# lbcb-sci/herro

Hardware: AMD Instinct MI355X
Metric: 4096-bp windows corrected/sec at batch=128 (higher is better)
Workload: dtype f16; 1 GPU; synthetic windows, 4096 bp, 32 overlaps each, batch=128, 1xMI355X per rank (BASELINE configs[2]); batch=128, window=4096, overlaps=32, batches_per_launch_group=32, streams_per_gpu=2, distinct_windows_cycled=16384, precision=5, total_windows=165760, strong_leg_windows=0

## Files before the change

### herro_amd/api.py

```python
from __future__ import annotations

import ctypes as C
import os
from dataclasses import dataclass

import numpy as np

_HERE = os.path.dirname(os.path.abspath(__file__))
LIB_PATH = os.environ.get("HERRO_LIB") or os.path.join(_HERE, "libherro_amd.so")
_LIB = None
DEFAULT_PRECISION = 4

EXPORTS = [
    "herro_version", "herro_create", "herro_destroy", "herro_last_error", "herro_set_stream", "herro_synchronize",
    "herro_encode_2bit", "herro_decode_2bit", "herro_set_reads", "herro_set_reads_packed", "herro_share_reads", "herro_load_model",
    "herro_set_precision", "herro_precision", "herro_clock_probe", "herro_calibration_error", "herro_debug_force_precision", "herro_model_describe", "herro_job_create", "herro_job_free", "herro_job_n_windows", "herro_job_skipped", "herro_job_featurize",
    "herro_job_infer", "herro_job_consensus", "herro_job_consensus_fetch", "herro_job_window_info", "herro_job_window_copy", "herro_job_window_logits",
    "herro_job_consensus_fasta", "herro_job_fasta", "herro_model_forward", "herro_timing_enable", "herro_timing_reset",
    "herro_timing_get", "herro_job_stats", "herro_debug_extract_windows",
    "herro_paf_parse", "herro_oec_read", "herro_paf_n_targets", "herro_paf_target_ids", "herro_paf_aln_off",
    "herro_paf_alignments", "herro_paf_free", "herro_name_index_create", "herro_name_index_free", "herro_paf_parse_indexed",
    "herro_oec_read_indexed", "herro_paf_parse_view", "herro_debug_host_ctx", "herro_debug_job_array", "herro_debug_tile_plan", "herro_debug_tile_plan_sib",
    "herro_debug_set_featurize_planes", "herro_debug_set_host_build", "herro_debug_job_dev_built", "herro_debug_job_rf", "herro_debug_job_cwd", "herro_debug_job_set_base_logits", "herro_debug_job_rf_fused", "herro_debug_job_rf_left", "herro_debug_e4m3", "herro_debug_sib_fault", "herro_debug_sib_retries", "herro_debug_base_row_votes", "herro_debug_vote5",
    "herro_pool_create", "herro_pool_destroy", "herro_pool_last_error", "herro_pool_size", "herro_pool_ctx", "herro_pool_set_reads", "herro_pool_load_model",
    "herro_pool_correct", "herro_pool_result", "herro_pool_groups_taken", "herro_pool_skipped", "herro_debug_pool_fake", "herro_job_create_status", "herro_host_register", "herro_host_unregister", "herro_debug_zero_copy_jobs",
    "herro_fastx_read", "herro_reads_count", "herro_reads_seq", "herro_reads_qual", "herro_reads_off", "herro_reads_ids",
    "herro_reads_descs", "herro_reads_free", "herro_write_window_features", "herro_job_write_features",
    "herro_paf_parse_coords", "herro_align_overlaps", "herro_aligned_alignments", "herro_aligned_scores", "herro_aligned_failed",
    "herro_aligned_free",
    "herro_align_overlaps_dev", "herro_aligned_dev_from_ops", "herro_aligned_dev_mirror", "herro_aligned_dev_n", "herro_aligned_dev_alignments", "herro_aligned_dev_scores",
    "herro_aligned_dev_n_ops", "herro_aligned_dev_failed", "herro_aligned_dev_cigar", "herro_aligned_dev_free", "herro_job_create_aligned",
    "herro_find_overlaps", "herro_overlaps_n", "herro_overlaps_n_targets", "herro_overlaps_target_ids", "herro_overlaps_aln_off",
    "herro_overlaps_alignments", "herro_overlaps_scores", "herro_overlaps_free", "herro_debug_sketch",
    "herro_extend_overlaps", "herro_extended_n", "herro_extended_alignments", "herro_extended_ext", "herro_extended_scores", "herro_extended_free",
    "herro_find_overlap_pairs", "herro_pairs_from_table", "herro_pairs_align", "herro_job_create_paired", "herro_pairs_n", "herro_pairs_primaries",
    "herro_pairs_chain_scores", "herro_pairs_ext", "herro_pairs_ext_scores", "herro_pairs_n_targets", "herro_pairs_target_ids", "herro_pairs_aln_off",
    "herro_pairs_rec_of_row", "herro_pairs_free",
    "herro_find_overlaps_core", "herro_find_overlap_pairs_core", "herro_pairs_from_table_core", "herro_pairs_n_rows",
]


class HerroError(RuntimeError):
    def __init__(self, code: int, msg: str):
        super().__init__(f"herro_amd error {code}: {msg}")
        self.code = code


class Alignment(C.Structure):
    _fields_ = [(n, C.c_uint32) for n in
                ("qid", "qlen", "qstart", "qend", "strand", "tid", "tlen", "tstart", "tend", "cigar_len")] + \
               [("cigar", C.c_void_p)]


ALN_DTYPE = np.dtype([("f", np.uint32, 10), ("p", np.uint64)], align=True)


def _aln_array(rows: np.ndarray, ncols: int = 9):
    n = len(rows)
    arr = (Alignment * max(n, 1))()
    view = np.frombuffer(arr, dtype=ALN_DTYPE, count=max(n, 1))
    if n:
        view["f"][:n, :ncols] = rows[:, :ncols]
    return arr, view


def _aln_rows(ptr, n: int, with_cigar_ptr: bool = False):
    rows, cig = np.zeros((n, 10), np.uint32), np.zeros(n, np.uint64)
    if n:
        view = np.frombuffer((Alignment * n).from_address(ptr), dtype=ALN_DTYPE, count=n)
        rows[:], cig[:] = view["f"], view["p"]
    return (rows, cig) if with_cigar_ptr else rows


def _job_or_raise(ctx: "Context", h, n_targets: int) -> "Job":
    if not h:
        msg = ctx._l.herro_last_error(ctx.h).decode(errors="replace")
        code = int(msg.rsplit("[code ", 1)[1].rstrip("]")) if "[code " in msg else -1
        raise HerroError(code, msg)
    return Job(ctx, h, n_targets)


PAIRS_NO_EXTEND = 1


class OverlapParams(C.Structure):
    _fields_ = [(n, C.c_uint32) for n in ("k", "w", "max_occ", "bandwidth", "max_gap", "min_score", "min_anchors", "reserved")]


class ExtendParams(C.Structure):
    _fields_ = [("zdrop", C.c_uint32), ("max_ext", C.c_uint32), ("reserved", C.c_uint32 * 2)]


class WindowInfo(C.Structure):
    _fields_ = [(n, C.c_uint32) for n in
                ("rid", "wid", "n_total_wins", "length", "n_alns", "n_overlaps", "n_supported", "win_len")]


def lib():
    global _LIB
    if _LIB is None:
        if not os.path.exists(LIB_PATH):
            raise RuntimeError(f"{LIB_PATH} not built — run __graft_entry__.build(); there is no CPU fallback")
        L = C.CDLL(LIB_PATH)
        vp, u32, u64, i32 = C.c_void_p, C.c_uint32, C.c_uint64, C.c_int
        L.herro_version.restype = C.c_char_p
# ... 106 lines not shown
        L.herro_aligned_free.argtypes = [vp]
        L.herro_align_overlaps_dev.argtypes = [vp, u32, vp, vp]
        L.herro_aligned_dev_from_ops.argtypes = [vp, u32, vp, vp, vp, vp]
        L.herro_aligned_dev_mirror.argtypes = [vp, vp, vp]
        for f in (L.herro_aligned_dev_n, L.herro_aligned_dev_failed):
            f.restype = u32
            f.argtypes = [vp]
        for f in (L.herro_aligned_dev_alignments, L.herro_aligned_dev_scores, L.herro_aligned_dev_n_ops):
            f.restype = vp
            f.argtypes = [vp]
        L.herro_aligned_dev_cigar.restype = C.c_int64
        L.herro_aligned_dev_cigar.argtypes = [vp, u32, vp, u64]
        L.herro_aligned_dev_free.restype = None
        L.herro_aligned_dev_free.argtypes = [vp]
        L.herro_job_create_aligned.restype = vp
        L.herro_job_create_aligned.argtypes = [vp, u32, vp, vp, vp, vp, u32]
        L.herro_find_overlaps.argtypes = [vp, vp, vp]
        for f in (L.herro_overlaps_n, L.herro_overlaps_n_targets):
            f.restype = u32
            f.argtypes = [vp]
        for f in (L.herro_overlaps_target_ids, L.herro_overlaps_aln_off, L.herro_overlaps_alignments, L.herro_overlaps_scores):
            f.restype = vp
            f.argtypes = [vp]
        L.herro_overlaps_free.restype = None
        L.herro_overlaps_free.argtypes = [vp]
        L.herro_extend_overlaps.argtypes = [vp, u32, vp, vp, vp]
        L.herro_extended_n.restype = u32
        L.herro_extended_n.argtypes = [vp]
        for f in (L.herro_extended_alignments, L.herro_extended_ext, L.herro_extended_scores):
            f.restype = vp
            f.argtypes = [vp]
        L.herro_extended_free.restype = None
        L.herro_extended_free.argtypes = [vp]
        L.herro_find_overlap_pairs.argtypes = [vp, vp, vp, u32, vp]
        L.herro_pairs_from_table.argtypes = [vp, u32, vp, vp, u32, vp, vp, vp, vp]
        L.herro_pairs_align.argtypes = [vp, vp, vp]
        L.herro_job_create_paired.restype = vp
        L.herro_job_create_paired.argtypes = [vp, vp, vp, u32]
        for f in (L.herro_pairs_n, L.herro_pairs_n_targets):
            f.restype = u32
            f.argtypes = [vp]
        for f in (L.herro_pairs_primaries, L.herro_pairs_chain_scores, L.herro_pairs_ext, L.herro_pairs_ext_scores, L.herro_pairs_target_ids,
                  L.herro_pairs_aln_off, L.herro_pairs_rec_of_row):
            f.restype = vp
            f.argtypes = [vp]
        L.herro_pairs_free.restype = None
        L.herro_pairs_free.argtypes = [vp]
        try:
            L.herro_find_overlaps_core.argtypes = [vp, vp, vp, vp]
            L.herro_find_overlap_pairs_core.argtypes = [vp, vp, vp, u32, vp, vp]
            L.herro_pairs_from_table_core.argtypes = [vp, u32, vp, vp, u32, vp, vp, u64, vp, vp]
            L.herro_pairs_n_rows.restype = u64
            L.herro_pairs_n_rows.argtypes = [vp]
        except AttributeError:
            if not os.environ.get("HERRO_LIB"):
                raise
        L.herro_debug_sketch.restype = C.c_int64
        L.herro_debug_sketch.argtypes = [vp, vp, vp, vp, vp, vp, u64]
        L.herro_debug_host_ctx.restype = vp
        L.herro_debug_host_ctx.argtypes = [u32, vp, vp]
        L.herro_debug_job_array.restype = C.c_int64
        L.herro_debug_job_array.argtypes = [vp, i32, vp, vp]
        L.herro_debug_set_featurize_planes.argtypes = [vp, i32]
        L.herro_debug_set_host_build.argtypes = [vp, i32]
        L.herro_debug_job_dev_built.argtypes = [vp]
        L.herro_debug_base_row_votes.argtypes = [vp, vp, vp, u32, vp, vp]
        L.herro_debug_vote5.restype = u32
        L.herro_debug_vote5.argtypes = [vp, u32]
        L.herro_debug_job_rf_fused.argtypes = [vp]
        L.herro_debug_job_rf_left.argtypes = [vp]
        L.herro_debug_sib_fault.argtypes = [vp]
        L.herro_debug_e4m3.argtypes = [C.c_float]
        L.herro_debug_e4m3.restype = C.c_uint32
        L.herro_debug_sib_retries.argtypes = [vp]
        L.herro_debug_job_rf.restype = C.c_int64
        L.herro_debug_job_rf.argtypes = [vp, u32, vp, u64]
        L.herro_debug_job_cwd.restype = C.c_int64
        L.herro_debug_job_cwd.argtypes = [vp, u32, vp, u64]
        L.herro_debug_job_set_base_logits.argtypes = [vp, vp, u64]
        L.herro_debug_tile_plan.restype = C.c_int64
        L.herro_debug_tile_plan.argtypes = [vp, u32, i32, u32, vp, vp, vp]
        L.herro_debug_tile_plan_sib.restype = i32
        L.herro_debug_tile_plan_sib.argtypes = [vp, u32, i32, u32, vp, vp, vp, vp]
        _LIB = L
    return _LIB


def encode_2bit(seq: bytes) -> np.ndarray:
    words = np.zeros((len(seq) + 31) // 32 + 1, np.uint64)
    buf = np.frombuffer(seq, np.uint8)
    n = lib().herro_encode_2bit(buf.ctypes.data if len(seq) else None, len(seq), words.ctypes.data)
    if n < 0:
        raise HerroError(int(n), "byte >= 128 in sequence")
    return words[:n].copy()


def decode_2bit(words: np.ndarray, length: int, start: int, end: int, rc: bool) -> bytes:
    words = np.ascontiguousarray(words, np.uint64)
    out = np.zeros(max(end - start, 0), np.uint8)
    r = lib().herro_decode_2bit(words.ctypes.data, length, start, end, int(rc), out.ctypes.data)
    if r:
        raise HerroError(r, "Out of bounds for 2-bit sequence decoding.")
    return out.tobytes()


def debug_extract_windows(row, cigar: bytes, n_windows: int, window_size: int) -> np.ndarray:
    a = Alignment()
    (a.qid, a.qlen, a.qstart, a.qend, a.strand, a.tid, a.tlen, a.tstart, a.tend) = (int(x) for x in row)
    buf = np.frombuffer(cigar + b"\0", np.uint8).copy()
    a.cigar_len, a.cigar = len(cigar), buf.ctypes.data
    out = np.zeros((65536, 8), np.uint64)
    err = C.create_string_buffer(512)
    n = lib().herro_debug_extract_windows(C.byref(a), n_windows, window_size, out.ctypes.data, len(out), err, 512)
    if n < 0:
        raise HerroError(int(n), err.value.decode())
    return out[:n].astype(np.int64)


def debug_tile_plan(counts, packed: bool = True, qmode: int = 0, n_cu: int = 256, bounds: bool = False):
    c = np.ascontiguousarray(counts, np.uint32)
    order = np.zeros(max(len(c), 1), np.uint32)
    n_half = C.c_uint32(0)
    tok = np.zeros(len(c) + 2, np.uint32)
    n = lib().herro_debug_tile_plan(c.ctypes.data, len(c), int(packed) | (qmode << 1), n_cu, order.ctypes.data, C.byref(n_half), tok.ctypes.data)
    if n < 0:
        raise HerroError(int(n), "herro_debug_tile_plan")
    out = (int(n), int(n_half.value), order[:len(c)]) if qmode else (int(n), order[:len(c)])
    return out + (tok[:int(n) + int(n_half.value) + 1],) if bounds else out


def debug_tile_plan_sib(counts, packed: bool = True, qmode: int = 1, n_cu: int = 256):
    c = np.ascontiguousarray(counts, np.uint32)
    order = np.zeros(max(len(c), 1), np.uint32)
    cap = int(((c.astype(np.int64) + 63) // 64).sum()) + 2
    n_tiles = np.zeros(3, np.uint32)
    tok = np.zeros(cap, np.uint32)
    grp = np.zeros(cap, np.uint32)
    rc = lib().herro_debug_tile_plan_sib(c.ctypes.data, len(c), int(packed) | (qmode << 1), n_cu, order.ctypes.data, n_tiles.ctypes.data, tok.ctypes.data, grp.ctypes.data)
    if rc < 0:
        raise HerroError(int(rc), "herro_debug_tile_plan_sib")
    nb, n64, n32 = (int(x) for x in n_tiles)
    return nb, n64, n32, order[:len(c)], tok[:nb + n64 + n32 + 1], grp[:nb]


class Pool:

    def __init__(self, device_ids, fake_us_per_aln=None):
        self._l = lib()
        if fake_us_per_aln is not None:
            us = np.ascontiguousarray(fake_us_per_aln, np.uint32)
            self.h = self._l.herro_debug_pool_fake(len(us), us.ctypes.data)
            self.n = len(us)
            if not self.h:
                raise HerroError(-1, "herro_debug_pool_fake")
            return
        ids = (C.c_int * len(device_ids))(*device_ids)
        self.h = self._l.herro_pool_create(ids, len(device_ids))
        if not self.h:
            raise HerroError(-1, self._l.herro_last_error(None).decode(errors="replace"))
        self.n = len(device_ids)

    def skipped(self) -> tuple[int, int]:
        a, t = C.c_uint64(0), C.c_uint64(0)
        self._chk(self._l.herro_pool_skipped(self.h, C.byref(a), C.byref(t)))
        return a.value, t.value

    def _chk(self, rc):
        if rc < 0:
            raise HerroError(int(rc), self._l.herro_pool_last_error(self.h).decode(errors="replace"))
        return rc

    def set_reads(self, seq, qual, off, name_class=None):
        seq, qual, off = np.ascontiguousarray(seq, np.uint8), np.ascontiguousarray(qual, np.uint8), np.ascontiguousarray(off, np.uint64)
        nc = None if name_class is None else np.ascontiguousarray(name_class, np.uint32)
        self._chk(self._l.herro_pool_set_reads(self.h, len(off) - 1, seq.ctypes.data, qual.ctypes.data, off.ctypes.data, None if nc is None else nc.ctypes.data))

    def load_model(self, path: str):
        self._chk(self._l.herro_pool_load_model(self.h, path.encode()))

    def set_precision(self, mode: int):
        for i in range(self.n):
            rc = self._l.herro_set_precision(self._l.herro_pool_ctx(self.h, i), mode)
            if rc:
                raise HerroError(rc, self._l.herro_last_error(self._l.herro_pool_ctx(self.h, i)).decode(errors="replace"))

    def correct(self, rids, rows, aln_off, cig_blob, cig_off, window_size: int, batch: int, read_ids, batch_mode: int = 1, group_targets: int = 1024):
        rids = np.ascontiguousarray(rids, np.uint32)
        aln_off = np.ascontiguousarray(aln_off, np.uint64)
        rows = np.ascontiguousarray(rows, np.uint32).reshape(-1, 10)
        blob = np.ascontiguousarray(cig_blob, np.uint8)
        m = len(rows)
        raw = np.zeros((max(m, 1), 12), np.uint32)
        if m:
            raw[:m, :10] = rows
            raw[:m, 10:12] = (np.asarray(cig_off, np.uint64) + np.uint64(blob.ctypes.data)).view(np.uint32).reshape(m, 2)
        names = (C.c_char_p * max(len(read_ids), 1))(*[r if isinstance(r, bytes) else r.encode() for r in read_ids])
        if len(read_ids) != len(rids):
            raise ValueError("one read id per target")
        n = self._chk(self._l.herro_pool_correct(self.h, len(rids), rids.ctypes.data, aln_off.ctypes.data, raw.ctypes.data, window_size, batch, batch_mode,
                                                 group_targets, names, None))
        ends_p = C.c_void_p()
        tp = self._l.herro_pool_result(self.h, C.byref(ends_p))
        text = np.ctypeslib.as_array((C.c_uint8 * n).from_address(tp)).copy() if n else np.zeros(0, np.uint8)
        ends = np.ctypeslib.as_array((C.c_uint64 * len(rids)).from_address(ends_p.value)).copy() if len(rids) else np.zeros(0, np.uint64)
        return text, ends

    def groups_taken(self):
        return [int(self._l.herro_pool_groups_taken(self.h, i)) for i in range(self.n)]

    def close(self):
        if self.h:
            self._l.herro_pool_destroy(self.h)
            self.h = None


@dataclass
class Window:
    info: WindowInfo
    bases: np.ndarray
    quals: np.ndarray
    sup_pos: np.ndarray
    sup_ins: np.ndarray
    qids: np.ndarray


# ... 212 lines not shown
            if n:
                ext[:] = np.ctypeslib.as_array(C.cast(self._l.herro_extended_ext(h), C.POINTER(C.c_uint32)), (n, 4))
                scores[:] = np.ctypeslib.as_array(C.cast(self._l.herro_extended_scores(h), C.POINTER(C.c_int32)), (n, 2))
        finally:
            self._l.herro_extended_free(h)
        return out, ext, scores

    def find_overlap_pairs(self, extend: bool = True, zdrop: int = 0, max_ext: int = 0, core=None, **params) -> "OverlapPairs":
        p = self._overlap_params(params)
        if not 0 <= int(zdrop) <= 0xFFFFFFFF or not 0 <= int(max_ext) <= 0xFFFFFFFF:
            raise HerroError(-1, "extend parameters: zdrop and max_ext are unsigned 32-bit values")
        e = ExtendParams(zdrop=int(zdrop), max_ext=int(max_ext))
        h = C.c_void_p()
        flags = 0 if extend else PAIRS_NO_EXTEND
        if core is None:
            self._chk(self._l.herro_find_overlap_pairs(self.h, C.byref(p), C.byref(e), flags, C.byref(h)))
        else:
            m = self._core_mask(core)
            self._chk(self._l.herro_find_overlap_pairs_core(self.h, C.byref(p), C.byref(e), flags, m.ctypes.data, C.byref(h)))
        return OverlapPairs(self, h)

    def pairs_from_table(self, primaries: np.ndarray, chain_scores, rids, aln_off, rec_of_row, n_rows: int | None = None) -> "OverlapPairs":
        rows = np.ascontiguousarray(primaries, np.uint32)
        n = len(rows)
        sc = None if chain_scores is None else np.ascontiguousarray(chain_scores, np.int32)
        rids = np.ascontiguousarray(rids, np.uint32)
        aln_off = np.ascontiguousarray(aln_off, np.uint64)
        rec_of_row = np.ascontiguousarray(rec_of_row, np.uint32)
        if len(aln_off) != len(rids) + 1 or len(rec_of_row) != (2 * n if n_rows is None else int(n_rows)) or (sc is not None and len(sc) != n):
            raise ValueError("aln_off has one entry per target + 1, rec_of_row two per primary (n_rows with n_rows), chain_scores one")
        arr, _ = _aln_array(rows)
        h = C.c_void_p()
        if n_rows is not None:
            self._chk(self._l.herro_pairs_from_table_core(self.h, n, C.byref(arr), None if sc is None else sc.ctypes.data, len(rids),
                                                          rids.ctypes.data if len(rids) else None, aln_off.ctypes.data, int(n_rows),
                                                          rec_of_row.ctypes.data if len(rec_of_row) else None, C.byref(h)))
            return OverlapPairs(self, h)
        self._chk(self._l.herro_pairs_from_table(self.h, n, C.byref(arr), None if sc is None else sc.ctypes.data, len(rids),
                                                 rids.ctypes.data if len(rids) else None, aln_off.ctypes.data,
                                                 rec_of_row.ctypes.data if n else None, C.byref(h)))
        return OverlapPairs(self, h)

    def create_job_paired(self, pairs: "OverlapPairs", m: "AlignedDev", window_size: int) -> "Job":
        h = self._l.herro_job_create_paired(self.h, pairs.h, m.h, window_size)
        return _job_or_raise(self, h, len(pairs.rids))

    def sketch(self, **params):
        p = self._overlap_params(params)
        n = self._l.herro_debug_sketch(self.h, C.byref(p), None, None, None, None, 0)
        if n < 0:
            self._chk(int(n))
        hs, rid, pos, st = np.zeros(n, np.uint64), np.zeros(n, np.uint32), np.zeros(n, np.uint32), np.zeros(n, np.uint8)
        if n:
            got = self._l.herro_debug_sketch(self.h, C.byref(p), hs.ctypes.data, rid.ctypes.data, pos.ctypes.data, st.ctypes.data, n)
            if got < 0:
                self._chk(int(got))
            assert got == n
        return hs, rid, pos, st

    def create_job_from_paf(self, paf: "Paf", window_size: int) -> "Job":
        h = self._l.herro_job_create(self.h, len(paf.targets), paf.targets.ctypes.data, paf.aln_off.ctypes.data,
                                     paf._alns_ptr, window_size)
        return _job_or_raise(self, h, len(paf.targets))

    def model_forward(self, bases: np.ndarray, quals: np.ndarray, lens: np.ndarray, indices: np.ndarray):
        bases = np.ascontiguousarray(bases, np.uint8)
        quals = np.ascontiguousarray(quals, np.uint8)
        lens = np.ascontiguousarray(lens, np.int32)
        indices = np.ascontiguousarray(indices, np.int32)
        B, L, R = bases.shape
        assert R == 31 and quals.shape == bases.shape
        N = int(lens.sum())
        info = np.zeros(N, np.float32)
        base = np.zeros((N, 5), np.float32)
        self._chk(self._l.herro_model_forward(self.h, B, L, bases.ctypes.data, quals.ctypes.data, lens.ctypes.data,
                                              indices.ctypes.data if N else None, info.ctypes.data, base.ctypes.data))
        return info, base

    def sib_fault(self):
        self._chk(self._l.herro_debug_sib_fault(self.h))

    def sib_retries(self) -> int:
        return int(self._l.herro_debug_sib_retries(self.h))

    def timing_enable(self, on: bool = True):
        self._chk(self._l.herro_timing_enable(self.h, int(on)))

    def timing_reset(self):
        self._chk(self._l.herro_timing_reset(self.h))

    def timing(self) -> dict[str, tuple[float, int]]:
        n = C.c_uint32(256)
        names = C.create_string_buffer(8192)
        ms = (C.c_double * 256)()
        calls = (C.c_uint64 * 256)()
        self._chk(self._l.herro_timing_get(self.h, names, 8192, ms, calls, C.byref(n)))
        nm = [x for x in names.value.decode().split("\n") if x]
        return {nm[i]: (ms[i], int(calls[i])) for i in range(min(n.value, len(nm)))}


class Job:
    def __init__(self, ctx: Context, h, n_targets: int):
        self.ctx, self.h, self.n_targets = ctx, h, n_targets
        self._l = ctx._l

    def close(self):
        if getattr(self, "h", None) and getattr(self.ctx, "h", None):
            self._l.herro_job_free(self.h)
        self.h = None

    __del__ = close

    @property
    def n_windows(self) -> int:
        return self._l.herro_job_n_windows(self.h)

    def skipped(self) -> tuple[int, int]:
        a, t = C.c_uint32(0), C.c_uint32(0)
        self.ctx._chk(self._l.herro_job_skipped(self.h, C.byref(a), C.byref(t)))
        return a.value, t.value

    def featurize(self):
        self.ctx._chk(self._l.herro_job_featurize(self.h))

    def infer(self, batch_size: int, batch_mode: int = 0):
        self.ctx._chk(self._l.herro_job_infer(self.h, batch_size, batch_mode))

    def consensus(self):
        self.ctx._chk(self._l.herro_job_consensus(self.h))

    def consensus_fetch(self) -> int:
        n = C.c_uint64(0)
        self.ctx._chk(self._l.herro_job_consensus_fetch(self.h, C.byref(n)))
        return n.value

    def info(self, w: int) -> WindowInfo:
        wi = WindowInfo()
        self.ctx._chk(self._l.herro_job_window_info(self.h, w, C.byref(wi)))
        return wi

    def window(self, w: int, encoded: bool = False) -> Window:
        wi = self.info(w)
        bases = np.zeros((wi.length, 31), np.uint8)
        quals = np.zeros((wi.length, 31), np.uint8)
        sp = np.zeros(wi.n_supported, np.uint16)
        si = np.zeros(wi.n_supported, np.uint8)
        qids = np.zeros(wi.n_overlaps, np.uint32)
        self.ctx._chk(self._l.herro_job_window_copy(self.h, w, int(encoded), bases.ctypes.data, quals.ctypes.data,
                                                    sp.ctypes.data, si.ctypes.data, qids.ctypes.data))
        return Window(wi, bases, quals, sp, si, qids)

    def logits(self, w: int):
        wi = self.info(w)
        info = np.zeros(wi.n_supported, np.float32)
        base = np.zeros((wi.n_supported, 5), np.float32)
        self.ctx._chk(self._l.herro_job_window_logits(self.h, w, info.ctypes.data, base.ctypes.data))
        return info, base

    def consensus_fasta(self, t: int, read_id: str, desc: str | None = None) -> str:
        cap = 1 << 24
        out = getattr(self, "_fasta_buf", None)
        if out is None:
            out = self._fasta_buf = C.create_string_buffer(cap)
        n = self._l.herro_job_consensus_fasta(self.h, t, read_id.encode(), None if desc is None else desc.encode(), out, cap)
        if n < 0:
            self.ctx._chk(int(n))
# ... 343 lines not shown
```

### herro_amd/csrc/api_ctx.h

```cpp
#pragma once
#include <hip/hip_runtime.h>

#include <atomic>
#include <condition_variable>
#include <cstdlib>
#include <functional>
#include <memory>
#include <mutex>
#include <string>
#include <thread>
#include <vector>

#include "../../include/herro_amd.h"
#include "job_dev.h"
#include "model_dev.h"

struct ErrSlot {
  std::mutex mu;
  std::string s;
  ErrSlot& operator=(const std::string& v) { std::lock_guard<std::mutex> lk(mu); s = v; return *this; }
  ErrSlot& operator=(const char* v) { std::lock_guard<std::mutex> lk(mu); s = v; return *this; }
  const char* c_str() const {
    thread_local std::string snap;
    { std::lock_guard<std::mutex> lk(const_cast<std::mutex&>(mu)); snap = s; }
    return snap.c_str();
  }
};

#define HIP_TRY(ctx, expr)                                                              \
  do {                                                                                  \
    hipError_t _e = (expr);                                                             \
    if (_e != hipSuccess) {                                                             \
      (ctx)->err = std::string(#expr) + ": " + hipGetErrorString(_e);                   \
      return HERRO_E_NO_DEVICE;                                                         \
    }                                                                                   \
  } while (0)

struct HostPool {
  std::vector<std::thread> th;
  std::mutex m;
  std::condition_variable cv, done_cv;
  const std::function<void(uint32_t)>* fn = nullptr;
  std::atomic<uint32_t> next{0};
  uint32_t n = 0, active = 0;
  uint64_t gen = 0;
  bool stop = false;
  explicit HostPool(uint32_t workers) {
    for (uint32_t i = 0; i < workers; i++) th.emplace_back([this] { loop(); });
  }
  ~HostPool() {
    { std::lock_guard<std::mutex> lk(m); stop = true; }
    cv.notify_all();
    for (auto& t : th) t.join();
  }
  void work() {
    for (;;) {
      const uint32_t i = next.fetch_add(1, std::memory_order_relaxed);
      if (i >= n) break;
      (*fn)(i);
    }
  }
  void loop() {
    uint64_t seen = 0;
    for (;;) {
      {
        std::unique_lock<std::mutex> lk(m);
        cv.wait(lk, [&] { return stop || gen != seen; });
        if (stop) return;
        seen = gen;
      }
      work();
      std::lock_guard<std::mutex> lk(m);
      if (--active == 0) done_cv.notify_one();
    }
  }
  std::mutex run_mu;
  void run(uint32_t count, const std::function<void(uint32_t)>& f) {
    if (count == 0) return;
    if (th.empty() || count == 1) { for (uint32_t i = 0; i < count; i++) f(i); return; }
    std::lock_guard<std::mutex> one_run(run_mu);
    {
      std::lock_guard<std::mutex> lk(m);
      fn = &f; n = count; next.store(0); active = (uint32_t)th.size(); gen++;
    }
    cv.notify_all();
    work();
    std::unique_lock<std::mutex> lk(m);
    done_cv.wait(lk, [&] { return active == 0; });
  }
};

struct Arena { void* p = nullptr; size_t cap = 0; };

struct herro_ctx {
  int device = 0;
  uint32_t n_cu = 256;
  hipStream_t own_stream = nullptr, stream = nullptr;
  ErrSlot err;
  uint32_t n_reads = 0;
  std::vector<uint32_t> read_len, name_class;
  std::vector<uint64_t> h_word_off, h_qual_off;
  bool host_only = false;
  bool lean = [] { const char* e = getenv("HERRO_FEATURIZE_PLANES"); return !e || atoi(e) == 0; }();
  bool tile_packing = herro::ab_env("HERRO_TILE_PACK", 1) != 0;
  uint64_t* d_words = nullptr;
  uint32_t* d_p0 = nullptr;
  uint32_t* d_p1 = nullptr;
  uint64_t* d_word_off = nullptr;
  uint8_t* d_qual = nullptr;
  uint64_t* d_qual_off = nullptr;
  double* d_ln = nullptr;
  uint32_t ln_n = 0;
  uint64_t read_bytes = 0, qual_bytes = 0, n_words = 0;
  std::shared_ptr<void> store_owner;
  bool has_model = false;
  herro::ModelDev M{};
  std::vector<void*> model_allocs;
  int precision = 1;
  bool precision_set = false;
  bool debug_force_precision = false;
  float wmax = 0.f;
  float calib[9] = {-1.f, -1.f, -1.f, -1.f, -1.f, -1.f, -1.f, -1.f, -1.f};
  std::string calib_note;
  herro::ModelScratch S{};
  uint32_t scratch_cap = 0;
  void* sib_kv = nullptr;
  void* sib_flag = nullptr;
  uint32_t sib_cap = 0;
  std::vector<void*> scratch_allocs;
  herro::KernelTimer timer;
  std::unique_ptr<HostPool> pool;
  std::mutex arena_mu;
  std::vector<Arena> free_scan, free_stage;
  hipStream_t prep_stream = nullptr;
  hipEvent_t prep_ev = nullptr;
  unsigned long long* d_prof = nullptr;
  bool dev_scan = true;
  bool dev_build = true;
  std::vector<Arena> free_dev, free_pin, free_small;
  std::atomic<uint32_t> live_jobs{0};
  uint64_t reads_gen = 0;
  uint32_t n_sib_retry = 0;
  std::vector<herro_job*> sib_suspects;
  std::atomic<int> n_pending{0};
  std::atomic<int> create_code{0};
};

HostPool& host_pool(herro_ctx* ctx);
```

### herro_amd/csrc/herro_api.hip

```cpp
#include <hip/hip_runtime.h>

#include <algorithm>
#include <cmath>
#include <cstdio>
#include <cstring>
#include <chrono>
#include <map>
#include <memory>
#include <string>
#include <atomic>
#include <condition_variable>
#include <functional>
#include <mutex>
#include <thread>
#include <unordered_map>
#include <vector>

#include "../../include/herro_amd.h"
#include "api_ctx.h"
#include "aligned_dev.h"
#include "host_cpus.h"
#include "job_dev.h"
#include "model_dev.h"
#include "windowing.hpp"
// ... 129 lines not shown
    const uint32_t want = env ? (uint32_t)std::max(1, atoi(env)) : std::min(std::min(std::max(std::thread::hardware_concurrency() / 4u, 1u), 64u), cpus);
    ctx->pool = std::make_unique<HostPool>(want - 1);
  }
  return *ctx->pool;
}

static Arena small_acquire(herro_ctx* ctx, size_t need) {
  {
    std::lock_guard<std::mutex> lk(ctx->arena_mu);
    size_t best = ctx->free_small.size();
    for (size_t i = 0; i < ctx->free_small.size(); i++)
      if (ctx->free_small[i].cap >= need && (best == ctx->free_small.size() || ctx->free_small[i].cap < ctx->free_small[best].cap)) best = i;
    if (best != ctx->free_small.size()) { Arena a = ctx->free_small[best]; ctx->free_small.erase(ctx->free_small.begin() + best); return a; }
  }
  Arena a;
  a.cap = need + need / 4 + 4096;
  if (hipMalloc(&a.p, a.cap) != hipSuccess) { a.p = nullptr; a.cap = 0; }
  return a;
}
static void small_release(herro_ctx* ctx, Arena& a) {
  if (!a.p) return;
  std::lock_guard<std::mutex> lk(ctx->arena_mu);
  if (ctx->free_small.size() < 24) ctx->free_small.push_back(a); else (void)hipFree(a.p);
  a = Arena{};
}

static Arena arena_acquire(herro_ctx* ctx, std::vector<Arena>& list, size_t need, int kind) {
  {
    std::lock_guard<std::mutex> lk(ctx->arena_mu);
    size_t best = list.size();
    for (size_t i = 0; i < list.size(); i++)
      if (list[i].cap >= need && (best == list.size() || list[i].cap < list[best].cap)) best = i;
    if (best != list.size()) { Arena a = list[best]; list.erase(list.begin() + best); return a; }
  }
  Arena a;
  a.cap = need + need / 8 + 4096;
  if (ctx->host_only) a.p = std::malloc(a.cap);
  else if (kind == 1) { if (hipMalloc(&a.p, a.cap) != hipSuccess) a.p = nullptr; }
  else if (hipHostMalloc(&a.p, a.cap, hipHostMallocDefault) != hipSuccess) a.p = nullptr;
  if (!a.p) a.cap = 0;
  return a;
}
struct ArenaReturn {
  herro_ctx* ctx; std::vector<Arena>* list; Arena* a; bool armed = true;
  ~ArenaReturn() {
    if (!armed || !a->p) return;
    std::lock_guard<std::mutex> lk(ctx->arena_mu);
    list->push_back(*a);
    *a = Arena{};
  }
};

static constexpr uint32_t FUSED_MAX_TOK = 64;
static constexpr uint32_t FUSED_HALF_TOK = 32;
static constexpr uint32_t FUSED_MAX_SIB = 8;
static std::vector<uint32_t> token_tiles(const std::vector<uint32_t>& tok_off, size_t w0 = 0, size_t w1 = ~size_t(0), uint32_t cap = FUSED_MAX_TOK) {
  w1 = std::min(w1, tok_off.size() - 1);
  if (w0 >= w1) return std::vector<uint32_t>();
  std::vector<uint32_t> t(1, tok_off[w0]);
  for (size_t w = w0; w < w1; w++) {
    if (tok_off[w + 1] - t.back() > cap) t.push_back(tok_off[w]);
  }
  if (tok_off[w1] > t.back()) t.push_back(tok_off[w1]);
  return t.size() > 1 ? t : std::vector<uint32_t>();
}

static void tile_pack_bins(const std::vector<uint32_t>& cnt, std::vector<std::vector<uint32_t>>& by, size_t left, uint32_t cap, std::vector<uint32_t>& order) {
  uint32_t top = cap;
  while (top && by[top].empty()) top--;
  while (left && top) {
    uint32_t room = cap, s = top;
    while (room) {
      s = std::min(s, room);
      while (s && by[s].empty()) s--;
      if (!s) break;
      order.push_back(by[s].back());
      by[s].pop_back();
      room -= s;
      left--;
    }
    while (top && by[top].empty()) top--;
  }
}
static std::vector<uint32_t> tile_pack_order(const std::vector<uint32_t>& cnt) {
  std::vector<std::vector<uint32_t>> by(FUSED_MAX_TOK + 1);
  for (size_t i = cnt.size(); i-- > 0;) by[std::min(cnt[i], FUSED_MAX_TOK)].push_back((uint32_t)i);
  std::vector<uint32_t> order;
  order.reserve(cnt.size());
  for (uint32_t i : by[0]) order.push_back(i);
  tile_pack_bins(cnt, by, cnt.size() - by[0].size(), FUSED_MAX_TOK, order);
  return order;
}

struct TilePlan { std::vector<uint32_t> order, tiles, tiles_q, tiles_b, grp; };
static TilePlan plan_tiles_small(const std::vector<uint32_t>& cnt, bool pack, int qmode, uint32_t n_cu, uint32_t n_busy = 0);
static TilePlan plan_tiles(const std::vector<uint32_t>& cnt, bool pack, int qmode, uint32_t n_cu) {
  std::vector<uint32_t> big, small;
  for (size_t i = 0; i < cnt.size(); i++) (cnt[i] > FUSED_MAX_TOK ? big : small).push_back((uint32_t)i);
  if (big.empty()) return plan_tiles_small(cnt, pack, qmode, n_cu);
  std::vector<std::vector<uint32_t>> by(FUSED_MAX_TOK + 1);
  if (pack) for (size_t k = small.size(); k-- > 0;) by[cnt[small[k]]].push_back(small[k]);
  std::vector<uint32_t> head, tiles_b(1, 0), grp;
  std::vector<char> taken(cnt.size(), 0);
  uint32_t tok = 0;
  for (uint32_t i : big) {
    const uint32_t k = (cnt[i] + FUSED_MAX_TOK - 1) / FUSED_MAX_TOK, g0 = (uint32_t)grp.size(), last = cnt[i] - (k - 1) * FUSED_MAX_TOK;
    head.push_back(i);
    for (uint32_t j = 0; j + 1 < k; j++) tiles_b.push_back(tok + (j + 1) * FUSED_MAX_TOK);
    tok += cnt[i];
    uint32_t room = FUSED_MAX_TOK - last, f = room;
    while (room) {
      f = std::min(f, room);
      while (f && by[f].empty()) f--;
      if (!f) break;
      const uint32_t w = by[f].back();
      by[f].pop_back();
      head.push_back(w);
      taken[w] = 1;
      tok += f;
      room -= f;
    }
    tiles_b.push_back(tok);
    for (uint32_t j = 0; j < k; j++) grp.push_back(g0 | (k << 20) | (last << 24));
  }
  std::vector<uint32_t> rest, rest_cnt;
  for (uint32_t i : small) if (!taken[i]) { rest.push_back(i); rest_cnt.push_back(cnt[i]); }
  TilePlan P = plan_tiles_small(rest_cnt, pack, qmode, n_cu, (uint32_t)grp.size());
  for (uint32_t& o : P.order) o = rest[o];
  for (uint32_t& t : P.tiles) t += tok;
  for (uint32_t& t : P.tiles_q) t += tok;
  P.order.insert(P.order.begin(), head.begin(), head.end());
  P.tiles_b.swap(tiles_b);
  P.grp.swap(grp);
  return P;
}
static TilePlan plan_tiles_small(const std::vector<uint32_t>& cnt, bool pack, int qmode, uint32_t n_cu, uint32_t n_busy) {
  TilePlan P;
  const size_t n = cnt.size();
  std::vector<uint32_t> tok_off(1, 0);
  auto finish = [&](size_t n_head) {
    tok_off.assign(1, 0);
    for (size_t k = 0; k < n; k++) tok_off.push_back(tok_off.back() + cnt[P.order[k]]);
    P.tiles = token_tiles(tok_off, 0, n_head, FUSED_MAX_TOK);
    P.tiles_q.clear();
    if (n_head < n) P.tiles_q = token_tiles(tok_off, n_head, n, FUSED_HALF_TOK);
  };
  if (qmode != 2) {
    if (pack) P.order = tile_pack_order(cnt);
    else { P.order.resize(n); for (size_t i = 0; i < n; i++) P.order[i] = (uint32_t)i; }
    finish(n);
    const size_t n64 = P.tiles.empty() ? 0 : P.tiles.size() - 1;
    const size_t rr = n_cu ? (n64 + n_busy) % n_cu : 0;
    if (qmode == 0 || rr == 0 || 2 * rr > n_cu) return P;
    const size_t r = std::min(rr, n64);
    if (r == 0) return P;
    const uint32_t cut_tok = P.tiles[n64 - r];
    size_t k0 = 0;
    while (tok_off[k0] < cut_tok) k0++;
    std::vector<uint32_t> keep, tail;
    for (size_t k = k0; k < n; k++) (cnt[P.order[k]] > FUSED_HALF_TOK ? keep : tail).push_back(P.order[k]);
    if (tail.empty()) return P;
    if (pack) {
      std::vector<std::vector<uint32_t>> by(FUSED_HALF_TOK + 1);
      for (size_t i = tail.size(); i-- > 0;) by[cnt[tail[i]]].push_back(tail[i]);
      std::vector<uint32_t> t2;
      for (uint32_t i : by[0]) t2.push_back(i);
      tile_pack_bins(cnt, by, tail.size() - by[0].size(), FUSED_HALF_TOK, t2);
      tail.swap(t2);
    }
    P.order.resize(k0);
    P.order.insert(P.order.end(), keep.begin(), keep.end());
    const size_t n_head = P.order.size();
    P.order.insert(P.order.end(), tail.begin(), tail.end());
    finish(n_head);
    return P;
  }
  P.order.reserve(n);
  if (!pack) {
    for (size_t i = 0; i < n; i++) if (cnt[i] > FUSED_HALF_TOK) P.order.push_back((uint32_t)i);
    const size_t n_head = P.order.size();
    for (size_t i = 0; i < n; i++) if (cnt[i] <= FUSED_HALF_TOK) P.order.push_back((uint32_t)i);
    finish(n_head);
    return P;
  }
  std::vector<std::vector<uint32_t>> by(FUSED_MAX_TOK + 1);
  for (size_t i = n; i-- > 0;) by[std::min(cnt[i], FUSED_MAX_TOK)].push_back((uint32_t)i);
  size_t small_left = 0;
  for (uint32_t s = 0; s <= FUSED_HALF_TOK; s++) small_left += by[s].size();
  for (uint32_t s = FUSED_MAX_TOK; s > FUSED_HALF_TOK; s--)
    while (!by[s].empty()) {
      P.order.push_back(by[s].back());
      by[s].pop_back();
      uint32_t room = FUSED_MAX_TOK - s, f = room;
      while (room) {
        f = std::min(f, room);
        while (f && by[f].empty()) f--;
        if (!f) break;
        P.order.push_back(by[f].back());
        by[f].pop_back();
        room -= f;
        small_left--;
      }
    }
  const size_t n_head = P.order.size();
  for (uint32_t i : by[0]) { P.order.push_back(i); small_left--; }
  tile_pack_bins(cnt, by, small_left, FUSED_HALF_TOK, P.order);
  finish(n_head);
  return P;
}

static uint32_t fused_tok_cap(const herro_ctx* ctx) {
  static const bool big = ab_env("HERRO_FUSED_BIG", 1) != 0;
  return (big && ctx->precision >= 4 && model_h_supported(ctx->M)) ? FUSED_MAX_TOK * FUSED_MAX_SIB : FUSED_MAX_TOK;
}
static int ensure_sib(herro_ctx* ctx, uint32_t n_tiles_b) {
  if (n_tiles_b <= ctx->sib_cap) return HERRO_OK;
  HIP_TRY(ctx, hipSetDevice(ctx->device));
  HIP_TRY(ctx, hipStreamSynchronize(ctx->stream));
  if (ctx->sib_kv) (void)hipFree(ctx->sib_kv);
  if (ctx->sib_flag) (void)hipFree(ctx->sib_flag);
  ctx->sib_kv = nullptr; ctx->sib_flag = nullptr; ctx->sib_cap = 0;
  const uint32_t cap = n_tiles_b + n_tiles_b / 2 + 8;
  if (hipMalloc(&ctx->sib_kv, (size_t)cap * 2 * 8 * 8 * 64 * 16) != hipSuccess || hipMalloc(&ctx->sib_flag, ((size_t)cap + 1) * 4) != hipSuccess ||
      hipMemset(ctx->sib_flag, 0, ((size_t)cap + 1) * 4) != hipSuccess) {
    if (ctx->sib_kv) (void)hipFree(ctx->sib_kv);
    ctx->sib_kv = nullptr;
    ctx->err = "out of device memory for the sibling-tile buffers";
    return HERRO_E_NO_DEVICE;
  }
  ctx->sib_cap = cap;
  ctx->S.sib_kv = (uint16_t*)ctx->sib_kv;
  ctx->S.sib_flag = (uint32_t*)ctx->sib_flag;
  ctx->S.sib_err = (uint32_t*)ctx->sib_flag + cap;
  return HERRO_OK;
}
static int check_sib(herro_ctx* ctx, herro_job* job) {
  if (!ctx->sib_flag) return HERRO_OK;
  uint32_t e = 0;
  HIP_TRY(ctx, hipMemcpyAsync(&e, (uint32_t*)ctx->sib_flag + ctx->sib_cap, 4, hipMemcpyDeviceToHost, ctx->stream));
  HIP_TRY(ctx, hipStreamSynchronize(ctx->stream));
  if (e) {
    for (herro_job* j : ctx->sib_suspects) j->sib_stale = true;
    (void)hipMemsetAsync((uint32_t*)ctx->sib_flag + ctx->sib_cap, 0, 4, ctx->stream);
  }
  ctx->sib_suspects.clear();
  if (job ? job->sib_stale : e != 0) {
    ctx->err = "fused stack: a sibling tile of a window above 64 informative rows never published its keys" + (e ? " (layer " + std::to_string(e - 1) + ")" : std::string()) + "; logits invalid";
    return HERRO_E_STATE;
  }
  return HERRO_OK;
}
__global__ void k_clock_probe(unsigned long long* out, uint32_t spin) {
  const unsigned long long c0 = clock64(), w0 = wall_clock64();
  uint32_t x = threadIdx.x;
  for (uint32_t i = 0; i < spin; i++) x = x * 1664525u + 1013904223u;
  const unsigned long long c1 = clock64(), w1 = wall_clock64();
  if (threadIdx.x == 0) { out[0] = c1 - c0; out[1] = w1 - w0; out[2] = x; }
}

static void run_model(herro_ctx* ctx, const BatchDev& B, bool tiled) {
  if (B.n_tok == 0) return;
  const int p = ctx->precision;
  if (!tiled) { launch_model(ctx->M, B, ctx->S, (p == 1 || p >= 4) ? 3 : p, ctx->stream, &ctx->timer); return; }
  if (p >= 4) launch_model_h(ctx->M, B, ctx->S, p == 4 ? 2 : (p == 6 ? 3 : (p == 7 ? 21 : (p == 8 ? 12 : 1))), ctx->stream, &ctx->timer);
  else launch_model(ctx->M, B, ctx->S, p, ctx->stream, &ctx->timer);
}

extern "C" {

const char* herro_version(void) { return "herro_amd 0.1 (gfx950)"; }

const char* herro_last_error(const herro_ctx* ctx) { return ctx ? ctx->err.c_str() : g_create_err.c_str(); }

herro_ctx* herro_create(int device_id) {
  int n = 0;
  hipError_t e = hipGetDeviceCount(&n);
  if (e != hipSuccess || n <= 0) {
    g_create_err = std::string("no HIP device: ") + (e != hipSuccess ? hipGetErrorString(e) : "device count 0");
    return nullptr;
  }
  if (device_id < 0 || device_id >= n) { g_create_err = "device id out of range"; return nullptr; }
  if ((e = hipSetDevice(device_id)) != hipSuccess) { g_create_err = hipGetErrorString(e); return nullptr; }
  auto ctx = std::make_unique<herro_ctx>();
  ctx->device = device_id;
  if ((e = hipStreamCreateWithFlags(&ctx->own_stream, hipStreamNonBlocking)) != hipSuccess) {
    g_create_err = hipGetErrorString(e);
    return nullptr;
  }
  ctx->stream = ctx->own_stream;
  {
    int cus = 0;
    if (hipDeviceGetAttribute(&cus, hipDeviceAttributeMultiprocessorCount, device_id) == hipSuccess && cus > 0) ctx->n_cu = (uint32_t)cus;
    int lo = 0, hi = 0;
    (void)hipDeviceGetStreamPriorityRange(&lo, &hi);
    if ((e = hipStreamCreateWithPriority(&ctx->prep_stream, hipStreamNonBlocking, hi)) != hipSuccess ||
        (e = hipEventCreateWithFlags(&ctx->prep_ev, hipEventDisableTiming | hipEventBlockingSync)) != hipSuccess) {
      g_create_err = hipGetErrorString(e);
      return nullptr;
    }
#ifdef HERRO_PROF_BUILD
    if (const char* pe = getenv("HERRO_PROF"); pe && atoi(pe)) {
      if (hipMalloc((void**)&ctx->d_prof, 256 * 32 * 8) == hipSuccess) (void)hipMemset(ctx->d_prof, 0, 256 * 32 * 8); else ctx->d_prof = nullptr;
    }
#endif
    ctx->dev_scan = ab_env("HERRO_HOST_SCAN", 0) == 0;
    { const char* e = getenv("HERRO_HOST_BUILD"); ctx->dev_build = !(e && atoi(e)); }
  }
  std::vector<double> ln(1u << 20);
  for (size_t k = 0; k < ln.size(); k++) ln[k] = std::log((double)k + 1.0);
  ctx->d_ln = dev_alloc_copy(ln, ctx->stream, e);
  if (e != hipSuccess) { g_create_err = hipGetErrorString(e); return nullptr; }
  if ((e = hipStreamSynchronize(ctx->stream)) != hipSuccess) { g_create_err = hipGetErrorString(e); return nullptr; }
  ctx->ln_n = (uint32_t)ln.size();
  return ctx.release();
}

static void free_all(std::vector<void*>& v) {
  for (void* p : v) if (p) (void)hipFree(p);
  v.clear();
}

void herro_destroy(herro_ctx* ctx) {
  if (!ctx) return;
  if (ctx->host_only) { for (Arena& a : ctx->free_pin) std::free(a.p); delete ctx; return; }
  (void)hipSetDevice(ctx->device);
  (void)hipDeviceSynchronize();
  if (ctx->d_prof) {
    std::vector<unsigned long long> raw(256 * 32);
    unsigned long long h[256] = {0};
    if (hipMemcpy(raw.data(), ctx->d_prof, raw.size() * 8, hipMemcpyDeviceToHost) == hipSuccess) {
      for (int i = 0; i < 256; i++) for (int sh = 0; sh < 32; sh++) h[i] += raw[(size_t)i * 32 + sh];
      for (int k = 0; k < 16; k++)
        if (h[k * 16 + 15]) {
          fprintf(stderr, "PROF kernel %d (%llu workgroups), cycles per workgroup by phase:", k, h[k * 16 + 15]);
          for (int ph = 0; ph < 15; ph++) if (h[k * 16 + ph]) fprintf(stderr, " %d:%.0f", ph, (double)h[k * 16 + ph] / (double)h[k * 16 + 15]);
          fprintf(stderr, "\n");
        }
    }
    (void)hipFree(ctx->d_prof);
#ifdef HERRO_PROF_BUILD
    model_h_prof_dump();
#endif
  }
  ctx->timer.reset();
  ctx->store_owner.reset();
  if (ctx->d_ln) (void)hipFree(ctx->d_ln);
  free_all(ctx->model_allocs);
// ... 1507 lines not shown

extern "C" {

int herro_job_infer(herro_job* job, uint32_t batch_size, int batch_mode) {
  if (!job || batch_size == 0) return HERRO_E_INVALID;
  herro_ctx* ctx = job->ctx;
  if (!ctx->has_model) { ctx->err = "no model loaded"; return HERRO_E_NO_MODEL; }
  ProfSpan span_(ctx, "infer");
  job->last_batch_size = batch_size; job->last_batch_mode = batch_mode;
  if (job->pending) { job->pending = false; ctx->n_pending--; }
  int rc = job_sync(job);
  if (rc) return rc;
  HIP_TRY(ctx, hipSetDevice(ctx->device));
  const uint32_t n = job->J.n_win;
  const uint64_t total_sup = job->sup_off[n];
  if (total_sup > 0xffffffffull / HERRO_ROWS) { ctx->err = "job too large (informative rows x 31 exceed 2^32: TokMeta::rf_idx is a 32-bit job-level index)"; return HERRO_E_UNSUPPORTED; }
  if ((rc = ensure_logits(job, total_sup))) return rc;
  if (ctx->M.pe_kind == 1)
    for (uint32_t w = 0; w < n; w++)
      if (job->h_nsup[w] && job->h_Lf[w] > ctx->M.pe_learned_rows) {
        ctx->err = "a window of " + std::to_string(job->h_Lf[w]) + " rows exceeds the model's learned position table (" + std::to_string(ctx->M.pe_learned_rows) + " rows): the archive would raise an index error";
        return HERRO_E_REFERENCE_PANIC;
      }
  bool rf_fused_ok = job->rf_fused && job->rf_total == total_sup && total_sup <= job->rf_fused_cap;
  uint32_t rf_left = 0;
  if (rf_fused_ok)
    for (uint32_t w = 0; w < n && rf_fused_ok; w++) {
      rf_fused_ok = job->h_nsup[w] == 0 || job->h_rfbase[w] != 0xffffffffu;
      rf_left += job->h_nsup[w] && job->h_rfbase[w] != 0xffffffffu && (job->h_rfbase[w] & 0x80000000u) ? 1u : 0u;
    }
  job->rf_fused_used = rf_fused_ok;
  job->rf_left_windows = rf_fused_ok ? rf_left : 0;
  job->rf_base.assign(n, 0);
  for (uint32_t w = 0; w < n; w++) job->rf_base[w] = rf_fused_ok ? (uint64_t)(job->h_rfbase[w] & 0x7fffffffu) : job->sup_off[w];
  job->batches.clear();
  auto flush = [&](std::vector<uint32_t>& cur) {
    if (cur.empty()) return;
    BatchPlan bp;
    bp.wins = cur;
    for (uint32_t w : cur) { bp.n_tok += job->h_nsup[w]; bp.lmax = std::max(bp.lmax, job->h_Lf[w]); }
    job->batches.push_back(std::move(bp));
    cur.clear();
  };
  std::vector<uint32_t> cur;
  if (batch_mode == 0) {
    for (uint32_t t = 0; t < job->n_targets; t++) {
      uint32_t seen = 0;
      for (uint32_t w = job->tgt_win_off[t]; w < job->tgt_win_off[t + 1]; w++) {
        if (job->h_nsup[w] > 0) cur.push_back(w);
        if (++seen == batch_size) { flush(cur); seen = 0; }
      }
      flush(cur);
    }
  } else {
    for (uint32_t w = 0; w < n; w++) {
      if (job->h_nsup[w] == 0) continue;
      cur.push_back(w);
      if (cur.size() == batch_size) flush(cur);
    }
    flush(cur);
  }
  const uint32_t TOK_CAP = 1u << 16;
  struct Group { size_t b0, b1; uint32_t n_win, n_tok; };
  std::vector<Group> groups;
  for (size_t bi = 0; bi < job->batches.size();) {
    Group g{bi, bi, 0, 0};
    while (g.b1 < job->batches.size() && (g.b1 == g.b0 || g.n_tok + job->batches[g.b1].n_tok <= TOK_CAP)) {
      g.n_win += (uint32_t)job->batches[g.b1].wins.size();
      g.n_tok += job->batches[g.b1].n_tok;
      g.b1++;
    }
    groups.push_back(g);
    bi = g.b1;
  }
  if (job->d_bdesc) HIP_TRY(ctx, hipEventSynchronize(job->ev_blob));
  std::vector<unsigned char>& blob = job->blob;
  blob.clear();
  auto put = [&](const void* p, size_t bytes) {
    const size_t o = (blob.size() + 15) & ~size_t(15);
    blob.resize(o + bytes);
    std::memcpy(blob.data() + o, p, bytes);
    return o;
  };
  struct Offs { size_t plane_off, plane_ld, len, lmax, tok_off, sup_off, out_off, rf_base, tiles, tiles_q, tiles_b, grp; uint32_t n_tiles, n_tiles_q, n_tiles_b, n_win, n_tok, max_win_tok; bool tiled; };
  std::vector<Offs> offs;
  uint32_t max_tok = 0, max_tiles_b = 0;
  const bool fused_mode = ctx->precision == 1 || ctx->precision >= 4;
  const uint32_t tok_cap = job->no_sib ? FUSED_MAX_TOK : fused_tok_cap(ctx);
  const int qmode = ctx->precision >= 4 ? model_h_half_tiles(ctx->M) : 0;
  for (auto& g : groups) {
    for (int part = 0; part < 2; part++) {
      std::vector<uint64_t> plane_off, sup_o, out_o, rfb;
      std::vector<uint32_t> ld, len, lmax, tok_off(1, 0), sel, sel_lmax, sel_cnt;
      for (size_t bi = g.b0; bi < g.b1; bi++) {
        const BatchPlan& bp = job->batches[bi];
        for (uint32_t w : bp.wins) {
          const bool large = fused_mode && job->h_nsup[w] > tok_cap;
          if ((int)large != part) continue;
          sel.push_back(w);
          sel_lmax.push_back(bp.lmax);
          sel_cnt.push_back(job->h_nsup[w]);
        }
      }
      const size_t B = sel.size();
      if (B == 0) continue;
      TilePlan plan;
      if (fused_mode && part == 0) plan = plan_tiles(sel_cnt, ctx->tile_packing, qmode, ctx->n_cu);
      const std::vector<uint32_t>& order = plan.order;
      plane_off.reserve(B); sup_o.reserve(B); out_o.reserve(B); ld.reserve(B); len.reserve(B); lmax.reserve(B); tok_off.reserve(B + 1);
      for (size_t k = 0; k < B; k++) {
        const size_t i = order.empty() ? k : order[k];
        const uint32_t w = sel[i];
        const WinDesc& wd = job->win[w];
        plane_off.push_back(wd.fin_off); ld.push_back(wd.lub); len.push_back(job->h_Lf[w]);
        lmax.push_back(sel_lmax[i]);
        tok_off.push_back(tok_off.back() + job->h_nsup[w]);
        sup_o.push_back(wd.row_off); out_o.push_back(job->sup_off[w]); rfb.push_back(job->rf_base[w]);
      }
      Offs o;
      o.n_win = (uint32_t)B; o.n_tok = tok_off.back(); o.tiled = fused_mode && part == 0;
      o.max_win_tok = *std::max_element(sel_cnt.begin(), sel_cnt.end());
      o.plane_off = put(plane_off.data(), B * 8); o.plane_ld = put(ld.data(), B * 4);
      o.len = put(len.data(), B * 4); o.lmax = put(lmax.data(), B * 4);
      o.tok_off = put(tok_off.data(), (B + 1) * 4);
      o.sup_off = put(sup_o.data(), B * 8); o.out_off = put(out_o.data(), B * 8); o.rf_base = put(rfb.data(), B * 8);
      o.n_tiles = plan.tiles.empty() ? 0u : (uint32_t)plan.tiles.size() - 1;
      o.tiles = put(plan.tiles.data(), plan.tiles.size() * 4);
      o.n_tiles_q = plan.tiles_q.empty() ? 0u : (uint32_t)plan.tiles_q.size() - 1;
      o.tiles_q = put(plan.tiles_q.data(), plan.tiles_q.size() * 4);
      o.n_tiles_b = (uint32_t)plan.grp.size();
      o.tiles_b = put(plan.tiles_b.data(), plan.tiles_b.size() * 4);
      o.grp = put(plan.grp.data(), plan.grp.size() * 4);
      offs.push_back(o);
      max_tok = std::max(max_tok, o.n_tok);
      max_tiles_b = std::max(max_tiles_b, o.n_tiles_b);
    }
  }
  const size_t supoff_at = put(job->sup_off.data(), ((size_t)n + 1) * 8);
  if (job->bdesc_cap < blob.size()) {
    if (job->d_bdesc) { HIP_TRY(ctx, hipStreamSynchronize(ctx->stream)); small_release(ctx, job->a_bdesc); job->d_bdesc = nullptr; }
    job->a_bdesc = small_acquire(ctx, blob.size() + blob.size() / 4 + 4096);
    if (!job->a_bdesc.p) { ctx->err = "out of device memory for the batch descriptors"; return HERRO_E_NO_DEVICE; }
    job->d_bdesc = job->a_bdesc.p;
    job->bdesc_cap = job->a_bdesc.cap;
  }
  HIP_TRY(ctx, hipMemcpyAsync(job->d_bdesc, blob.data(), blob.size(), hipMemcpyHostToDevice, ctx->stream));
  HIP_TRY(ctx, hipEventRecord(job->ev_blob, ctx->stream));
  job->d_supoff_blob = (const uint64_t*)((const unsigned char*)job->d_bdesc + supoff_at);
  rc = ensure_scratch(ctx, max_tok);
  if (rc) return rc;
  if (max_tiles_b && (rc = ensure_sib(ctx, max_tiles_b))) return rc;
  const uint32_t rf_half = 2 * (ctx->M.h.kw / 2);
  const bool rf_compact = job->d_rfq && 2 * rf_half + 1 <= 8;
  const bool rfq_there = rf_compact && ((rf_fused_ok && job->rf_fused_half == rf_half) ||
                                        (job->rfq_spec && job->rfq_spec_half == rf_half && job->rfq_spec_cap >= total_sup));
  if (!rf_compact && !job->tokens_full && !groups.empty()) {
    launch_full_tokens(job->J, ctx->stream, &ctx->timer);
    job->tokens_full = true;
  }
  if (!(job->quals_full && !rf_compact) && !groups.empty() && !rfq_there)
    launch_rf_quals(job->J, rf_half, job->d_supoff_blob, rf_compact ? job->d_rfq : nullptr, job->logit_cap, job->lean, ctx->stream, &ctx->timer);
  else if (rf_compact && rf_fused_ok && job->rf_fused_half == rf_half && job->rf_left_windows && !groups.empty())
    launch_rf_quals(job->J, rf_half, job->d_supoff_blob, job->d_rfq, job->logit_cap, job->lean, ctx->stream, &ctx->timer, true);
  for (const Offs& o : offs) {
    const unsigned char* base = (const unsigned char*)job->d_bdesc;
    BatchDev B{};
    B.n_win = o.n_win; B.n_tok = o.n_tok; B.max_win_tok = o.max_win_tok;
    B.plane_off = (const uint64_t*)(base + o.plane_off);
    B.plane_ld = (const uint32_t*)(base + o.plane_ld);
    B.len = (const uint32_t*)(base + o.len);
    B.lmax = (const uint32_t*)(base + o.lmax);
    B.tok_off = (const uint32_t*)(base + o.tok_off);
    B.sup_off = (const uint64_t*)(base + o.sup_off);
    B.out_off = (const uint64_t*)(base + o.out_off);
    B.rf_base = (const uint64_t*)(base + o.rf_base);
    B.n_tiles = o.n_tiles;
    B.tile_tok0 = (const uint32_t*)(base + o.tiles);
    B.n_tiles_q = o.n_tiles_q;
    B.tile_tok0_q = (const uint32_t*)(base + o.tiles_q);
    B.n_tiles_b = o.n_tiles_b;
    B.tile_tok0_b = (const uint32_t*)(base + o.tiles_b);
    B.tile_grp = (const uint32_t*)(base + o.grp);
    B.planes_b = job->J.fin_b; B.planes_q = job->J.fin_q; B.sup_row = job->J.sup_row;
    B.rf_q = rf_compact ? job->d_rfq : nullptr;
    B.out_info = job->d_info; B.out_base = job->d_base;
    if (o.tiled && o.n_tiles_b && std::find(ctx->sib_suspects.begin(), ctx->sib_suspects.end(), job) == ctx->sib_suspects.end()) ctx->sib_suspects.push_back(job);
    run_model(ctx, B, o.tiled);
  }
  HIP_TRY(ctx, hipGetLastError());
  job->sib_stale = false;
  job->inferred = true;
  job->logits_on_host = false;
  job->consensus_done = false;
  return HERRO_OK;
}

int herro_job_consensus(herro_job* job) {
  if (!job) return HERRO_E_INVALID;
  herro_ctx* ctx = job->ctx;
  ProfSpan span_(ctx, "consensus");
  int rc = job_sync(job);
  if (rc) return rc;
  HIP_TRY(ctx, hipSetDevice(ctx->device));
  const uint32_t n = job->J.n_win;
  if (job->sup_off.back() > 0 && !job->inferred) { ctx->err = "herro_job_infer has not run"; return HERRO_E_STATE; }
  const uint64_t* d_so = job->d_supoff_blob;
  if (!job->inferred || !d_so) {
    if (!job->d_supoff) {
      job->a_supoff = small_acquire(ctx, std::max<uint64_t>(n, 1) * 8);
      if (!job->a_supoff.p) { ctx->err = "out of device memory"; return HERRO_E_NO_DEVICE; }
      job->d_supoff = (uint64_t*)job->a_supoff.p;
    }
    if (!job->d_base) {
      job->a_logits = small_acquire(ctx, 512);
      if (!job->a_logits.p) { ctx->err = "out of device memory"; return HERRO_E_NO_DEVICE; }
      job->d_info = (float*)job->a_logits.p;
      job->d_base = (float*)((unsigned char*)job->a_logits.p + 256);
      job->logit_cap = 1;
    }
    if (n) HIP_TRY(ctx, hipMemcpyAsync(job->d_supoff, job->sup_off.data(), n * 8ull, hipMemcpyHostToDevice, ctx->stream));
    d_so = job->d_supoff;
  }
  launch_consensus(job->J, d_so, job->d_base, job->lean, ctx->stream, &ctx->timer);
  HIP_TRY(ctx, hipGetLastError());
  job->consensus_done = true;
  job->consensus_on_host = false;
  return HERRO_OK;
}

int herro_job_window_info(herro_job* job, uint32_t w, herro_window_info* info) {
  if (!job || !info || w >= job->win.size()) return HERRO_E_INVALID;
  int rc = job_sync(job);
  if (rc) return rc;
  const WinDesc& wd = job->win[w];
  info->rid = wd.rid; info->wid = wd.wid; info->n_total_wins = wd.n_wids;
  info->length = job->h_Lf[w];
  info->n_overlaps = job->h_nkept[w];
  info->n_alns = std::min<uint32_t>(job->h_nkept[w], 30);
  info->n_supported = job->h_nsup[w];
  info->win_len = wd.win_len;
  return HERRO_OK;
}

static int fetch_planes(herro_job* job, uint32_t w, std::vector<uint8_t>& pb, std::vector<uint8_t>* pq) {
  herro_ctx* ctx = job->ctx;
  const WinDesc& wd = job->win[w];
  const size_t bytes = (size_t)HERRO_ROWS * wd.lub;
  pb.resize(bytes);
  if (!job->tokens_full) {
    launch_full_tokens(job->J, ctx->stream, nullptr);
    HIP_TRY(ctx, hipGetLastError());
    HIP_TRY(ctx, hipStreamSynchronize(ctx->stream));
    job->tokens_full = true;
  }
  HIP_TRY(ctx, hipMemcpy(pb.data(), job->J.fin_b + wd.fin_off, bytes, hipMemcpyDeviceToHost));
  if (pq) {
    if (!job->quals_full) {
      launch_full_quals(job->J, ctx->stream);
      HIP_TRY(ctx, hipGetLastError());
      HIP_TRY(ctx, hipStreamSynchronize(ctx->stream));
// ... 291 lines not shown
  if (rc) return rc;
  int64_t n = 0;
  std::vector<uint8_t> bases, quals, sins;
  std::vector<uint16_t> spos;
  std::vector<uint32_t> qids;
  std::vector<const char*> ids;
  for (uint32_t t = 0; t < job->n_targets; t++) {
    for (uint32_t w = job->tgt_win_off[t]; w < job->tgt_win_off[t + 1]; w++) {
      const WinDesc& wd = job->win[w];
      const uint32_t L = job->h_Lf[w], ns = job->h_nsup[w], nk = job->h_nkept[w];
      bases.resize((size_t)L * HERRO_ROWS); quals.resize(bases.size());
      spos.resize(ns); sins.resize(ns); qids.resize(nk); ids.resize(nk);
      if ((rc = herro_job_window_copy(job, w, 0, bases.data(), quals.data(), spos.data(), sins.data(), qids.data()))) return rc;
      for (uint32_t k = 0; k < nk; k++) {
        if (qids[k] >= ctx->n_reads || !read_names[qids[k]]) { ctx->err = "read name missing"; return HERRO_E_INVALID; }
        ids[k] = read_names[qids[k]];
      }
      if (wd.rid >= ctx->n_reads || !read_names[wd.rid]) { ctx->err = "read name missing"; return HERRO_E_INVALID; }
      const std::string dir = std::string(base_dir) + "/" + read_names[wd.rid];
      if ((rc = herro_write_window_features(dir.c_str(), wd.wid, ids.data(), nk, bases.data(), quals.data(), L, spos.data(), sins.data(), ns))) {
        ctx->err = "cannot write features under " + dir;
        return rc;
      }
      n++;
    }
  }
  return n;
}

int herro_model_forward(herro_ctx* ctx, uint32_t B, uint32_t L, const uint8_t* bases, const uint8_t* quals,
                        const int32_t* lens, const int32_t* indices, float* info_logits, float* bases_logits) {
  if (!ctx || !bases || !quals || !lens) return HERRO_E_INVALID;
  if (!ctx->has_model) { ctx->err = "no model loaded"; return HERRO_E_NO_MODEL; }
  HIP_TRY(ctx, hipSetDevice(ctx->device));
  uint64_t N = 0;
  std::vector<uint32_t> tok_off(B + 1, 0), srow;
  for (uint32_t b = 0; b < B; b++) {
    if (lens[b] < 0) return HERRO_E_INVALID;
    tok_off[b + 1] = tok_off[b] + (uint32_t)lens[b];
    N += (uint64_t)lens[b];
  }
  if (N && (!indices || !info_logits || !bases_logits)) return HERRO_E_INVALID;
  srow.resize(N);
  for (uint64_t i = 0; i < N; i++) {
    if (indices[i] < 0 || (uint32_t)indices[i] >= L) { ctx->err = "index out of range"; return HERRO_E_REFERENCE_PANIC; }
    if (ctx->M.pe_kind == 1 && (uint32_t)indices[i] >= ctx->M.pe_learned_rows) { ctx->err = "index beyond the model's learned position table"; return HERRO_E_REFERENCE_PANIC; }
    srow[i] = (uint32_t)indices[i];
  }
  if (N == 0) return HERRO_OK;
  const uint64_t cells = (uint64_t)B * L * HERRO_ROWS;
  std::vector<void*> tmp;
  auto A = [&](uint64_t bytes) -> void* { void* p = nullptr; if (hipMalloc(&p, std::max<uint64_t>(bytes, 16)) == hipSuccess) tmp.push_back(p); return p; };
  auto done = [&](int code) { for (void* p : tmp) (void)hipFree(p); return code; };
  hipStream_t st = ctx->stream;
  hipError_t e = hipSuccess;
  auto up = [&](const void* src, uint64_t bytes) -> void* {
    void* p = A(bytes);
    if (p && bytes && e == hipSuccess) e = hipMemcpyAsync(p, src, bytes, hipMemcpyHostToDevice, st);
    return p;
  };
  uint8_t* d_src_b = (uint8_t*)up(bases, cells); uint8_t* d_src_q = (uint8_t*)up(quals, cells);
  uint8_t* d_pb = (uint8_t*)A(cells + 16); uint8_t* d_pq = (uint8_t*)A(cells + 16);
  uint32_t* d_sr = (uint32_t*)up(srow.data(), N * 4);
  float* d_info = (float*)A(N * 4); float* d_base = (float*)A(N * 20);
  if (!d_src_b || !d_src_q || !d_pb || !d_pq || !d_sr || !d_info || !d_base) { ctx->err = "out of device memory"; return done(HERRO_E_NO_DEVICE); }
  launch_transpose_blr(d_src_b, d_pb, B, L, st);
  launch_transpose_blr(d_src_q, d_pq, B, L, st);
  int rc = HERRO_OK;
  if ((rc = ensure_scratch(ctx, (uint32_t)N))) return done(rc);
  struct Part { std::vector<uint64_t> plane_off, sup_off, out_off; std::vector<uint32_t> ld, len, lmax, tok_off; TilePlan plan; };
  Part parts[2];
  const bool fused_mode = ctx->precision == 1 || ctx->precision >= 4;
  for (int part = 0; part < 2; part++) {
    Part& P = parts[part];
    P.tok_off.assign(1, 0);
    const bool tiled = fused_mode && part == 0;
    std::vector<uint32_t> sel, sel_cnt;
    for (uint32_t b = 0; b < B; b++) {
      const bool large = fused_mode && (uint32_t)lens[b] > fused_tok_cap(ctx);
      if ((int)large != part) continue;
      sel.push_back(b);
      sel_cnt.push_back((uint32_t)lens[b]);
    }
    if (tiled) P.plan = plan_tiles(sel_cnt, ctx->tile_packing, ctx->precision >= 4 ? model_h_half_tiles(ctx->M) : 0, ctx->n_cu);
    const std::vector<uint32_t>& order = P.plan.order;
    for (size_t k = 0; k < sel.size(); k++) {
      const uint32_t b = sel[order.empty() ? k : order[k]];
      P.plane_off.push_back((uint64_t)b * HERRO_ROWS * L); P.ld.push_back(L); P.len.push_back(L); P.lmax.push_back(L);
      P.sup_off.push_back(tok_off[b]); P.out_off.push_back(tok_off[b]);
      P.tok_off.push_back(P.tok_off.back() + (uint32_t)lens[b]);
    }
    const size_t nb = P.plane_off.size();
    if (nb == 0 || P.tok_off.back() == 0) continue;
    BatchDev bd{};
    bd.n_win = (uint32_t)nb; bd.n_tok = P.tok_off.back(); bd.max_win_tok = *std::max_element(sel_cnt.begin(), sel_cnt.end());
    bd.plane_off = (const uint64_t*)up(P.plane_off.data(), nb * 8); bd.plane_ld = (const uint32_t*)up(P.ld.data(), nb * 4);
    bd.len = (const uint32_t*)up(P.len.data(), nb * 4); bd.lmax = (const uint32_t*)up(P.lmax.data(), nb * 4);
    bd.tok_off = (const uint32_t*)up(P.tok_off.data(), (nb + 1) * 4);
    bd.sup_off = (const uint64_t*)up(P.sup_off.data(), nb * 8); bd.out_off = (const uint64_t*)up(P.out_off.data(), nb * 8);
    bd.tile_tok0 = (const uint32_t*)up(P.plan.tiles.data(), P.plan.tiles.size() * 4);
    bd.n_tiles = P.plan.tiles.empty() ? 0u : (uint32_t)P.plan.tiles.size() - 1;
    bd.tile_tok0_q = (const uint32_t*)up(P.plan.tiles_q.data(), P.plan.tiles_q.size() * 4);
    bd.n_tiles_q = P.plan.tiles_q.empty() ? 0u : (uint32_t)P.plan.tiles_q.size() - 1;
    bd.tile_tok0_b = (const uint32_t*)up(P.plan.tiles_b.data(), P.plan.tiles_b.size() * 4);
    bd.tile_grp = (const uint32_t*)up(P.plan.grp.data(), P.plan.grp.size() * 4);
    bd.n_tiles_b = (uint32_t)P.plan.grp.size();
    if (bd.n_tiles_b && (rc = ensure_sib(ctx, bd.n_tiles_b))) { (void)hipStreamSynchronize(st); return done(rc); }
    bd.planes_b = d_pb; bd.planes_q = d_pq; bd.rf_q = nullptr; bd.sup_row = d_sr; bd.out_info = d_info; bd.out_base = d_base;
    if (!bd.plane_off || !bd.plane_ld || !bd.len || !bd.lmax || !bd.tok_off || !bd.sup_off || !bd.out_off || !bd.tile_tok0 || !bd.tile_tok0_q || !bd.tile_tok0_b || !bd.tile_grp || e != hipSuccess) {
      ctx->err = e != hipSuccess ? hipGetErrorString(e) : "out of device memory";
      (void)hipStreamSynchronize(st);
      return done(HERRO_E_NO_DEVICE);
    }
    run_model(ctx, bd, tiled);
  }
  if (e == hipSuccess) e = hipStreamSynchronize(st);
  if (e == hipSuccess) e = hipGetLastError();
  if (e != hipSuccess) { ctx->err = hipGetErrorString(e); return done(HERRO_E_NO_DEVICE); }
  ctx->timer.collect();
  if ((rc = check_sib(ctx, nullptr))) return done(rc);
  HIP_TRY(ctx, hipMemcpy(info_logits, d_info, N * 4, hipMemcpyDeviceToHost));
  HIP_TRY(ctx, hipMemcpy(bases_logits, d_base, N * 20, hipMemcpyDeviceToHost));
  return done(HERRO_OK);
}

herro_ctx* herro_debug_host_ctx(uint32_t n_reads, const uint32_t* read_len, const uint32_t* name_class) {
  auto ctx = new herro_ctx();
  ctx->host_only = true;
  ctx->n_reads = n_reads;
  ctx->read_len.assign(read_len, read_len + n_reads);
  ctx->name_class.resize(n_reads);
  for (uint32_t i = 0; i < n_reads; i++) ctx->name_class[i] = name_class ? name_class[i] : i;
  ctx->h_word_off.assign(n_reads + 1, 0);
  ctx->h_qual_off.assign(n_reads + 1, 0);
  for (uint32_t i = 0; i < n_reads; i++) {
    ctx->h_word_off[i + 1] = ctx->h_word_off[i] + ((uint64_t)read_len[i] + 31) / 32;
    ctx->h_qual_off[i + 1] = ctx->h_qual_off[i] + read_len[i];
  }
  return ctx;
}

int herro_debug_base_row_votes(const uint8_t* counts, const uint8_t* split, const uint8_t* target, uint32_t n, uint8_t* sup, uint8_t* vote) {
  if (!counts || !target || !sup || !vote) return HERRO_E_INVALID;
  for (uint32_t g0 = 0; g0 < n; g0 += 32) {
    const uint32_t m = std::min(32u, n - g0);
    uint32_t a0[5] = {0, 0, 0, 0, 0}, a1[5] = {0, 0, 0, 0, 0}, b0[5] = {0, 0, 0, 0, 0}, b1[5] = {0, 0, 0, 0, 0}, tsym[4] = {0, 0, 0, 0};
    const uint32_t vm = m == 32 ? 0xffffffffu : ((1u << m) - 1u);
    for (uint32_t i = 0; i < m; i++) {
      if (target[g0 + i] > 3) return HERRO_E_INVALID;
      tsym[target[g0 + i]] |= 1u << i;
    }
    for (int q = 0; q < 5; q++)
      for (uint32_t k = 0; k < 255; k++) {
        uint32_t xa = 0, xb = 0;
        for (uint32_t i = 0; i < m; i++) {
          const uint32_t c = counts[(size_t)(g0 + i) * 5 + q], s = split ? std::min<uint32_t>(split[(size_t)(g0 + i) * 5 + q], c) : 0u;
          if (k < c - s) xa |= 1u << i;
          if (k < s) xb |= 1u << i;
        }
        if (!xa && !xb) break;
        sat2_add(a0[q], a1[q], xa);
        sat2_add(b0[q], b1[q], xb);
      }
    for (int q = 0; q < 5; q++) sat2_merge(a0[q], a1[q], b0[q], b1[q]);
    const RowVotes r = base_row_votes(a0, a1, tsym, vm);
    for (uint32_t i = 0; i < m; i++) {
      sup[g0 + i] = (uint8_t)((r.sup >> i) & 1u);
      vote[g0 + i] = (uint8_t)(((r.v0 >> i) & 1u) | (((r.v1 >> i) & 1u) << 1) | (((r.v2 >> i) & 1u) << 2));
    }
  }
  return HERRO_OK;
}

uint32_t herro_debug_vote5(const uint32_t* c5, uint32_t tb) {
  const uint32_t c[5] = {c5[0], c5[1], c5[2], c5[3], c5[4]};
  return vote5(c, tb);
}

int herro_debug_set_featurize_planes(herro_ctx* ctx, int on) {
  if (!ctx) return HERRO_E_INVALID;
  ctx->lean = on == 0;
  return HERRO_OK;
}

int herro_debug_sib_fault(herro_ctx* ctx) {
  if (!ctx) return HERRO_E_INVALID;
  if (int rc = ensure_sib(ctx, 1)) return rc;
  const uint32_t one = 1;
  HIP_TRY(ctx, hipMemcpyAsync((uint32_t*)ctx->sib_flag + ctx->sib_cap, &one, 4, hipMemcpyHostToDevice, ctx->stream));
  HIP_TRY(ctx, hipStreamSynchronize(ctx->stream));
  return HERRO_OK;
}
int herro_debug_sib_retries(const herro_ctx* ctx) { return ctx ? (int)ctx->n_sib_retry : HERRO_E_INVALID; }

int herro_clock_probe(herro_ctx* ctx, double* shader_mhz) {
  if (!ctx || !shader_mhz) return HERRO_E_INVALID;
  HIP_TRY(ctx, hipSetDevice(ctx->device));
  int wall_khz = 0;
  HIP_TRY(ctx, hipDeviceGetAttribute(&wall_khz, hipDeviceAttributeWallClockRate, ctx->device));
  unsigned long long* d = nullptr;
  HIP_TRY(ctx, hipMalloc((void**)&d, 32));
  hipLaunchKernelGGL(k_clock_probe, dim3(1), dim3(64), 0, ctx->stream, d, 20000u);
  unsigned long long h[3] = {0, 0, 0};
  hipError_t e = hipMemcpyAsync(h, d, sizeof h, hipMemcpyDeviceToHost, ctx->stream);
  if (e == hipSuccess) e = hipStreamSynchronize(ctx->stream);
  (void)hipFree(d);
  HIP_TRY(ctx, e);
  *shader_mhz = h[1] ? (double)h[0] / (double)h[1] * (double)wall_khz * 1e-3 : 0.0;
  return HERRO_OK;
}
uint32_t herro_debug_e4m3(float x) { return f32_to_e4m3(x); }
int herro_debug_job_rf_fused(const herro_job* job) { return job && job->inferred ? (job->rf_fused_used ? 1 : 0) : HERRO_E_STATE; }
int herro_debug_job_rf_left(const herro_job* job) { return job && job->inferred ? (int)job->rf_left_windows : HERRO_E_STATE; }

int64_t herro_debug_job_rf(herro_job* job, uint32_t w, uint8_t* out, uint64_t cap) {
  if (!job || w >= job->win.size() || !out) return HERRO_E_INVALID;
  herro_ctx* ctx = job->ctx;
  if (!job->inferred || !job->d_rfq) { ctx->err = "herro_job_infer has not run"; return HERRO_E_STATE; }
  const uint64_t n = (uint64_t)job->h_nsup[w] * HERRO_ROWS;
  if (n * 16 > cap) { ctx->err = "output buffer too small"; return HERRO_E_INVALID; }
  HIP_TRY(ctx, hipSetDevice(ctx->device));
  HIP_TRY(ctx, hipStreamSynchronize(ctx->stream));
  if (n) HIP_TRY(ctx, hipMemcpy(out, job->d_rfq + job->rf_base[w] * HERRO_ROWS * 16, n * 16, hipMemcpyDeviceToHost));
  return (int64_t)n;
}

int64_t herro_debug_job_cwd(herro_job* job, uint32_t ow, uint32_t* out, uint64_t cap) {
  if (!job || !out) return HERRO_E_INVALID;
  herro_ctx* ctx = job->ctx;
  if (ctx->host_only || !job->featurized) { ctx->err = "herro_job_featurize has not run"; return HERRO_E_STATE; }
  if (ow >= job->J.n_ow || cap < job->J.nw) { ctx->err = "overlap-window index out of range or output buffer too small"; return HERRO_E_INVALID; }
  HIP_TRY(ctx, hipSetDevice(ctx->device));
  HIP_TRY(ctx, hipStreamSynchronize(ctx->stream));
  HIP_TRY(ctx, hipMemcpy(out, job->J.cwd + (uint64_t)ow * job->J.nw, (size_t)job->J.nw * 4, hipMemcpyDeviceToHost));
  return (int64_t)job->J.nw;
}

int herro_debug_job_set_base_logits(herro_job* job, const float* base, uint64_t n_rows) {
  if (!job || (n_rows && !base)) return HERRO_E_INVALID;
  herro_ctx* ctx = job->ctx;
  int rc = job_sync(job);
  if (rc) return rc;
  if (!job->inferred) { ctx->err = "herro_job_infer has not run"; return HERRO_E_STATE; }
  const uint64_t tot = job->sup_off.back();
  if (n_rows != tot) { ctx->err = "n_rows " + std::to_string(n_rows) + " != the job's informative rows " + std::to_string(tot); return HERRO_E_INVALID; }
  if ((rc = logits_to_host(job))) return rc;
  if (tot) {
    std::memcpy(job->h_base.data(), base, tot * 20);
    HIP_TRY(ctx, hipSetDevice(ctx->device));
    HIP_TRY(ctx, hipMemcpy(job->d_base, base, tot * 20, hipMemcpyHostToDevice));
  }
  job->consensus_done = false;
  job->consensus_on_host = false;
  return HERRO_OK;
}

int64_t herro_debug_job_array(herro_job* job, int which, const void** ptr, uint32_t* elem_bytes) {
  if (!job || !ptr || !elem_bytes) return HERRO_E_INVALID;
  switch (which) {
    case 0:
      *elem_bytes = 4;
      if (job->scan.p) {
        job->dbg_ops.resize(job->scan_ops);
        if (hipSetDevice(job->ctx->device) != hipSuccess || hipDeviceSynchronize() != hipSuccess ||
            hipMemcpy(job->dbg_ops.data(), job->scan.p, job->scan_ops * 4, hipMemcpyDeviceToHost) != hipSuccess) return HERRO_E_NO_DEVICE;
        *ptr = job->dbg_ops.data();
        return (int64_t)job->dbg_ops.size();
      }
      *ptr = job->ops.data();
      return (int64_t)job->ops.size();
    case 1:
      *elem_bytes = sizeof(OwDesc);
      if (job->dev_built) {
        job->dbg_ow.resize(job->J.n_ow);
        if (hipSetDevice(job->ctx->device) != hipSuccess || hipDeviceSynchronize() != hipSuccess ||
            (job->J.n_ow && hipMemcpy(job->dbg_ow.data(), job->J.ow, (size_t)job->J.n_ow * sizeof(OwDesc), hipMemcpyDeviceToHost) != hipSuccess)) return HERRO_E_NO_DEVICE;
        *ptr = job->dbg_ow.data();
        return (int64_t)job->dbg_ow.size();
      }
      *ptr = job->ow.data();
      return (int64_t)job->ow.size();
    case 2: *ptr = job->win.data(); *elem_bytes = sizeof(WinDesc); return (int64_t)job->win.size();
    case 3:
    case 4:
      *elem_bytes = 4;
      if (job->dev_built) {
        std::vector<uint32_t>& v = which == 3 ? job->dbg_tw : job->dbg_tr;
        v.resize(job->J.n_tiles);
        if (hipSetDevice(job->ctx->device) != hipSuccess || hipDeviceSynchronize() != hipSuccess ||
            (job->J.n_tiles && hipMemcpy(v.data(), which == 3 ? job->J.tile_win : job->J.tile_r0, (size_t)job->J.n_tiles * 4, hipMemcpyDeviceToHost) != hipSuccess)) return HERRO_E_NO_DEVICE;
        *ptr = v.data();
        return (int64_t)v.size();
      }
      *ptr = which == 3 ? job->tile_win.data() : job->tile_r0.data();
      return (int64_t)(which == 3 ? job->tile_win.size() : job->tile_r0.size());
    case 5: *ptr = job->tgt_win_off.data(); *elem_bytes = 4; return (int64_t)job->tgt_win_off.size();
    default: return HERRO_E_INVALID;
  }
}

int64_t herro_debug_tile_plan(const uint32_t* cnt, uint32_t n, int packed, uint32_t n_cu, uint32_t* order, uint32_t* n_half, uint32_t* tile_tok) {
  if (!cnt || !order) return HERRO_E_INVALID;
  std::vector<uint32_t> c(cnt, cnt + n);
  for (uint32_t v : c) if (v == 0 || v > FUSED_MAX_TOK) return HERRO_E_INVALID;
  const TilePlan P = plan_tiles(c, (packed & 1) != 0, (packed >> 1) & 3, n_cu);
  for (uint32_t i = 0; i < n; i++) order[i] = P.order[i];
  for (size_t k = 0; k + 1 < P.tiles.size(); k++) if (P.tiles[k + 1] - P.tiles[k] > FUSED_MAX_TOK) return HERRO_E_STATE;
  for (size_t k = 0; k + 1 < P.tiles_q.size(); k++) if (P.tiles_q[k + 1] - P.tiles_q[k] > FUSED_HALF_TOK) return HERRO_E_STATE;
  if (!P.tiles.empty() && !P.tiles_q.empty() && P.tiles.back() != P.tiles_q.front()) return HERRO_E_STATE;
  const size_t n64 = P.tiles.empty() ? 0 : P.tiles.size() - 1, n32 = P.tiles_q.empty() ? 0 : P.tiles_q.size() - 1;
  if (n_half) *n_half = (uint32_t)n32;
  if (tile_tok) {
    size_t k = 0;
    for (size_t i = 0; i < n64; i++) tile_tok[k++] = P.tiles[i];
    for (size_t i = 0; i < n32; i++) tile_tok[k++] = P.tiles_q[i];
    tile_tok[k] = n32 ? P.tiles_q.back() : (n64 ? P.tiles.back() : 0);
  }
  return (int64_t)n64;
}

int herro_debug_tile_plan_sib(const uint32_t* cnt, uint32_t n, int packed, uint32_t n_cu, uint32_t* order, uint32_t* n_tiles, uint32_t* tile_tok, uint32_t* grp) {
  if (!cnt || !order || !n_tiles) return HERRO_E_INVALID;
  std::vector<uint32_t> c(cnt, cnt + n);
  for (uint32_t v : c) if (v == 0 || v > FUSED_MAX_TOK * FUSED_MAX_SIB) return HERRO_E_INVALID;
  const TilePlan P = plan_tiles(c, (packed & 1) != 0, (packed >> 1) & 3, n_cu);
  for (uint32_t i = 0; i < n; i++) order[i] = P.order[i];
  const size_t nb = P.grp.size(), n64 = P.tiles.empty() ? 0 : P.tiles.size() - 1, n32 = P.tiles_q.empty() ? 0 : P.tiles_q.size() - 1;
  if (nb && P.tiles_b.size() != nb + 1) return HERRO_E_STATE;
  n_tiles[0] = (uint32_t)nb; n_tiles[1] = (uint32_t)n64; n_tiles[2] = (uint32_t)n32;
  if (tile_tok) {
    size_t k = 0;
    uint32_t end = 0;
    for (size_t i = 0; i < nb; i++) tile_tok[k++] = P.tiles_b[i];
    if (nb) end = P.tiles_b.back();
    for (size_t i = 0; i < n64; i++) tile_tok[k++] = P.tiles[i];
    if (n64) end = P.tiles.back();
    for (size_t i = 0; i < n32; i++) tile_tok[k++] = P.tiles_q[i];
    if (n32) end = P.tiles_q.back();
    tile_tok[k] = end;
  }
  if (grp) for (size_t i = 0; i < nb; i++) grp[i] = P.grp[i];
  return HERRO_OK;
}

int64_t herro_debug_extract_windows(const herro_alignment* a, uint32_t n_windows, uint32_t W, uint64_t* out,
                                    uint64_t cap, char* err, uint64_t err_cap) {
  std::vector<uint32_t> ops;
  std::vector<HostOw> hows;
  BuildError be;
  if (!a || !parse_cigar(a->cigar, a->cigar_len, ops, be) || !window_alignment(ops, *a, W, n_windows, hows, be)) {
    if (err && err_cap) { std::strncpy(err, a ? be.msg.c_str() : "null", err_cap - 1); err[err_cap - 1] = 0; }
    return a ? be.code : HERRO_E_INVALID;
  }
  if (hows.size() > cap) return HERRO_E_INVALID;
  for (size_t k = 0; k < hows.size(); k++) {
    uint64_t* o = out + 8 * k;
    o[0] = hows[k].win; o[1] = hows[k].tstart; o[2] = hows[k].qstart; o[3] = hows[k].qend;
    o[4] = hows[k].op_lo; o[5] = hows[k].op_hi; o[6] = hows[k].start_off; o[7] = hows[k].end_off;
  }
  return (int64_t)hows.size();
}

int herro_timing_enable(herro_ctx* ctx, int on) { if (!ctx) return HERRO_E_INVALID; ctx->timer.on = on != 0; return HERRO_OK; }
int herro_timing_reset(herro_ctx* ctx) {
  if (!ctx) return HERRO_E_INVALID;
  HIP_TRY(ctx, hipStreamSynchronize(ctx->stream));
  ctx->timer.reset();
  return HERRO_OK;
}
int herro_timing_get(herro_ctx* ctx, char* names, uint64_t cap, double* ms, uint64_t* calls, uint32_t* n) {
  if (!ctx || !n) return HERRO_E_INVALID;
  HIP_TRY(ctx, hipStreamSynchronize(ctx->stream));
  ctx->timer.collect();
  std::string s;
  uint32_t k = 0;
  for (auto& nm : ctx->timer.order) {
    if (k < *n) {
      if (ms) ms[k] = ctx->timer.acc[nm].first;
      if (calls) calls[k] = ctx->timer.acc[nm].second;
    }
    s += nm;
    s += "\n";
    k++;
  }
  if (names && cap) { std::strncpy(names, s.c_str(), cap - 1); names[cap - 1] = 0; }
  *n = k;
  return HERRO_OK;
}

int herro_job_stats(herro_job* job, uint64_t* out) {
  if (!job || !out) return HERRO_E_INVALID;
  int rc = job_sync(job);
  if (rc) return rc;
  uint64_t sumL = 0, sumS = 0, nz = 0;
  for (size_t w = 0; w < job->win.size(); w++) { sumL += job->h_Lf[w]; sumS += job->h_nsup[w]; nz += job->h_nsup[w] > 0; }
  out[0] = job->alg_read_bytes; out[1] = job->alg_op_bytes; out[2] = 2ull * HERRO_ROWS * sumL;
  out[3] = sumL; out[4] = sumS; out[5] = nz;
  return HERRO_OK;
}

herro_job* herro_job_create_aligned(herro_ctx* ctx, uint32_t n_targets, const uint32_t* rids, const uint64_t* aln_off, const uint32_t* rec,
// ... 51 lines not shown
```

### herro_amd/csrc/model_dev.h

```cpp
#pragma once
#include <hip/hip_runtime.h>
#include <stdint.h>

#include "job_dev.h"

namespace herro {

struct ModelHyper {
  uint32_t magic;
  uint32_t version;
  uint32_t rows;
  uint32_t kw;
  uint32_t c1, c2;
  uint32_t d_model, n_heads, d_ff, n_layers;
  uint32_t n_tensors;
  float ln_eps;
};

struct Weight {
  const float* f32 = nullptr;
  const uint16_t* hi = nullptr;
  const uint16_t* lo = nullptr;
  const uint16_t* phi = nullptr;
  const uint16_t* plo = nullptr;
  const uint16_t* h16 = nullptr;
  const uint16_t* l16 = nullptr;
  const uint16_t* ph16 = nullptr;
  const uint8_t* p8 = nullptr;
  uint32_t s8 = 127;
  const float* bias = nullptr;
  uint32_t K = 0, N = 0;
};

struct LayerW {
  const float *ln1_g, *ln1_b, *ln2_g, *ln2_b;
  Weight qkv, proj, ff1, ff2;
};

struct ModelDev {
  ModelHyper h;
  const float* t1;
  const float* wq1;
  const float* b1;
  Weight conv1g;
  Weight conv2;
  Weight fc;
  const float* pe_div;
  const float* pe_tab;
  uint32_t pe_rows;
  LayerW layer[16];
  const float *lnf_g, *lnf_b;
  Weight heads;
  uint32_t act;
  uint32_t norm_first;
  uint32_t pe_kind;
  uint32_t final_norm;
  const float* pe_learned;
  uint32_t pe_learned_rows;
};
inline bool model_default_variant(const ModelDev& M) { return M.act == 0 && M.norm_first == 1 && M.pe_kind == 0 && M.final_norm == 1; }

struct BatchDev {
  uint32_t n_win;
  uint32_t n_tok;
  uint32_t max_win_tok;
  const uint64_t* plane_off;
  const uint32_t* plane_ld;
  const uint32_t* len;
  const uint32_t* lmax;
  const uint32_t* tok_off;
  const uint64_t* sup_off;
  const uint64_t* out_off;
  const uint64_t* rf_base;
  const uint8_t* planes_b;
  const uint8_t* planes_q;
  const uint8_t* rf_q;
  const uint32_t* sup_row;
  uint32_t n_tiles;
  const uint32_t* tile_tok0;
  uint32_t n_tiles_q;
  const uint32_t* tile_tok0_q;
  uint32_t n_tiles_b;
  const uint32_t* tile_tok0_b;
  const uint32_t* tile_grp;
  float* out_info;
  float* out_base;
};

struct __attribute__((aligned(16))) TokMeta {
  uint64_t plane_off;
  uint32_t plane_ld;
  uint32_t tok_row;
  uint32_t len, lmax;
  uint32_t rf_idx;
  uint32_t pad1;
};

struct __attribute__((aligned(16))) TokCv {
  uint64_t plane_off;
  uint32_t ld_d1;
  uint32_t row_ok;
  uint32_t rf_idx;
  uint32_t mk0, dt0, dq0;
};

struct ModelScratch {
  uint32_t* tok_win;
  uint32_t* tok_row;
  uint64_t* tok_out;
  TokMeta* tok_meta;
  TokCv* tok_cv;
  float* y1;
  float* y2;
  float* x;
  float* hbuf;
  float* qkv;
  float* att;
  float* ff;
  float* logits;
  uint16_t *y1_hi, *y1_lo;
  uint16_t *y2_hi, *y2_lo;
  uint16_t *h_hi, *h_lo;
  uint16_t *att_hi, *att_lo;
  uint16_t *ff_hi, *ff_lo;
  uint16_t* sib_kv;
  uint32_t* sib_flag;
  uint32_t* sib_err;
};

void launch_model(const ModelDev& M, const BatchDev& B, const ModelScratch& S, int precision,
                  hipStream_t st, KernelTimer* tm);
bool model_h_supported(const ModelDev& M);
bool model_h_conv_supported(const ModelDev& M);
void launch_front_generic(const ModelDev& M, const BatchDev& B, const ModelScratch& S, hipStream_t st, KernelTimer* tm);
bool model_h_f8_supported(const ModelDev& M);
int model_h_half_tiles(const ModelDev& M);
void launch_model_h(const ModelDev& M, const BatchDev& B, const ModelScratch& S, int terms, hipStream_t st, KernelTimer* tm);
void launch_pe_table(const float* pe_div, float* tab, uint32_t rows, uint32_t d_model, hipStream_t st);
#ifdef HERRO_PROF_BUILD
void model_h_prof_dump();
#endif
void launch_transpose_blr(const uint8_t* src, uint8_t* dst, uint32_t B, uint32_t L, hipStream_t st);

}
```

### herro_amd/csrc/model_h.hip

```cpp
#include <hip/hip_runtime.h>
#include <stdint.h>

#include <algorithm>
#include <cstdlib>
#include <mutex>
#include <set>
#include <type_traits>
#include <utility>

#include "model_dev.h"

namespace herro {

namespace {

typedef float f32x4 __attribute__((ext_vector_type(4)));
typedef _Float16 half8 __attribute__((ext_vector_type(8)));
typedef _Float16 half2v __attribute__((ext_vector_type(2)));
typedef float float2v __attribute__((ext_vector_type(2)));

__device__ __forceinline__ float norm_qual_h(uint32_t q) {
  const float QS = (float)(2.0 / 93.0);
  const float QO = (float)(2.0 * 33.0 / 93.0 + 1.0);
  return __fsub_rn(__fmul_rn(QS, (float)q), QO);
// ... 521 lines not shown
      __builtin_amdgcn_sched_barrier(0);
    }
    if (TERMS == 3 && k == 6) { wload8(cur, 1, w8b); __builtin_amdgcn_sched_barrier(0); }
    if (TERMS == 3 && k == 7) {
#pragma unroll
      for (int pt = 0; pt < PT; pt++) xb[pt] = rd8(0, pt);
      __builtin_amdgcn_sched_barrier(0);
    }
    if (AHEAD2) {
      if (k + 2 < 8) rd(sh, k + 2, xm);
      __builtin_amdgcn_sched_barrier(0);
      if (k < 4) mm8(xh, wa[k]); else mm8(xh, wb[k - 4]);
      __builtin_amdgcn_sched_barrier(0);
#pragma unroll
      for (int pt = 0; pt < PT; pt++) { xh[pt] = xn[pt]; xn[pt] = xm[pt]; }
      continue;
    }
    if (TERMS == 2 && !(dbg_rd && (k & 1))) rd(sl, k, xl);
    __builtin_amdgcn_sched_barrier(0);
    if (!(dbg_mm && (k & 1))) { if (k < 4) mm8(xh, wa[k]); else mm8(xh, wb[k - 4]); }
    __builtin_amdgcn_sched_barrier(0);
    if (k < 7 && !(dbg_rd && !(k & 1))) rd(sh, k + 1, xn);
    __builtin_amdgcn_sched_barrier(0);
    if (TERMS == 2 && !(dbg_mm && (k & 1))) {
      if (k < 4) mm8(xl, wa[k]); else mm8(xl, wb[k - 4]);
      __builtin_amdgcn_sched_barrier(0);
    }
#pragma unroll
    for (int pt = 0; pt < PT; pt++) xh[pt] = xn[pt];
  }
  if constexpr (TERMS == 3) {
    v8i xc[PT];
#pragma unroll
    for (int pt = 0; pt < PT; pt++) xc[pt] = rd8(1, pt);
    __builtin_amdgcn_sched_barrier(0);
#pragma unroll
    for (int pt = 0; pt < PT; pt++) {
#pragma unroll
      for (int jt = 0; jt < 2; jt++) if (!(HERRO_LP_DBG & 8)) acc[pt][jt] = mma8(w8a[jt], xb[pt], acc[pt][jt], cur.s8);
      __builtin_amdgcn_sched_barrier(0);
    }
#pragma unroll
    for (int pt = 0; pt < PT; pt++) asm volatile("" : "+v"(acc[pt][0]), "+v"(acc[pt][1]), "+v"(w8b[0]), "+v"(w8b[1]));
#pragma unroll
    for (int pt = 0; pt < PT; pt++) {
#pragma unroll
      for (int jt = 0; jt < 2; jt++) if (!(HERRO_LP_DBG & 8)) acc[pt][jt] = mma8(w8b[jt], xc[pt], acc[pt][jt], cur.s8);
      __builtin_amdgcn_sched_barrier(0);
    }
  }
}

constexpr int PAR_LN1G = 0, PAR_LN1B = 256, PAR_LN2G = 512, PAR_LN2B = 768, PAR_BQKV = 1024, PAR_BPROJ = 1792, PAR_BFF2 = 2048, PAR_BFF1 = 2304;
constexpr int PAR_MAX_FF = 2048;
constexpr int PAR_FLOATS = PAR_BFF1 + PAR_MAX_FF;

#ifdef HERRO_PROF_BUILD
__device__ unsigned long long g_lp_prof[16];
#define LP_BEGIN() unsigned long long _lp_t = (tid == 0 && (blockIdx.x & 15u) == 0) ? __builtin_readcyclecounter() : 0ull
#define LP_MARK(ph)                                                                      \
  do {                                                                                   \
    if (tid == 0 && (blockIdx.x & 15u) == 0) {                                           \
      const unsigned long long _n = __builtin_readcyclecounter();                        \
      atomicAdd(&g_lp_prof[ph], _n - _lp_t);                                             \
      if ((ph) == 0) atomicAdd(&g_lp_prof[15], 1ull);                                    \
      _lp_t = __builtin_readcyclecounter();                                              \
    }                                                                                    \
  } while (0)
#else
#define LP_BEGIN() do { } while (0)
#define LP_MARK(ph) do { } while (0)
#endif

template <int TERMS, int PT, bool SIB = false>
__global__ __launch_bounds__(512) void k_layers_p(ModelDev M, BatchDev B, ModelScratch S) {
  static_assert(!SIB || PT == 4, "sibling tiles are 64-token tiles");
  constexpr int TP = TERMS == 21 ? 2 : (TERMS == 12 ? 1 : TERMS);
  constexpr int TF = TERMS == 21 ? 1 : (TERMS == 12 ? 2 : TERMS);
  const bool big = SIB && blockIdx.x < B.n_tiles_b;
  const uint32_t bt = SIB ? (big ? blockIdx.x : blockIdx.x - B.n_tiles_b) : blockIdx.x;
  constexpr int HLT = 16 * PT;
  extern __shared__ __attribute__((aligned(16))) unsigned char smem[];
  uint16_t* s_hh = reinterpret_cast<uint16_t*>(smem);
  uint16_t* s_hl = s_hh + HLT * 256;
  uint16_t* s_ah = s_hl + HLT * 256;
  uint16_t* s_al = s_ah + HLT * 256;
  float* s_red = reinterpret_cast<float*>(s_al + HLT * 256);
  uint32_t* s_win = reinterpret_cast<uint32_t*>(s_red + 2 * 8 * HLT);
  float* s_par = reinterpret_cast<float*>(s_win + HLT);
  const uint32_t tid = threadIdx.x, lane = tid & 63, wave = __builtin_amdgcn_readfirstlane(tid >> 6);
  LP_BEGIN();
  uint32_t fr = lane & 15, fg = lane >> 4;
  const uint32_t* tile_tok0 = PT == 4 ? (big ? B.tile_tok0_b : B.tile_tok0) : B.tile_tok0_q;
  const uint32_t t0 = tile_tok0[bt], nt = tile_tok0[bt + 1] - t0;
  const uint32_t grp = big ? B.tile_grp[bt] : 0u;
  const uint32_t cw = wave * 32;
  const float eps = M.h.ln_eps;
  const uint32_t n_layers = M.h.n_layers, d_ff = M.h.d_ff;
#define RELAUNDER() asm volatile("" : "+v"(fr), "+v"(fg))

  if (tid < HLT) s_win[tid] = tid < nt ? S.tok_win[t0 + tid] : 0xffffff00u + tid;
  f32x4 xr[PT][2];
#define XQ(pt, q) xr[pt][(q) >> 2][(q) & 3]
  half8 wa[4][2];
  wload4(wstream(M.layer[0].qkv, cw, 0, lane), 0, wa);

  auto lds8 = [&](uint32_t o, float (&v)[8]) {
    const float4 a = *reinterpret_cast<const float4*>(s_par + o), b = *reinterpret_cast<const float4*>(s_par + o + 4);
    v[0] = a.x; v[1] = a.y; v[2] = a.z; v[3] = a.w; v[4] = b.x; v[5] = b.y; v[6] = b.z; v[7] = b.w;
  };
  auto stage_params = [&](const LayerW& L) {
    uint32_t tid_ = threadIdx.x;
    asm volatile("" : "+v"(tid_));
    const uint32_t tid = tid_;
    for (uint32_t e = tid; e < 256; e += 512) {
      s_par[PAR_LN1G + e] = L.ln1_g[e]; s_par[PAR_LN1B + e] = L.ln1_b[e];
      s_par[PAR_LN2G + e] = L.ln2_g[e]; s_par[PAR_LN2B + e] = L.ln2_b[e];
      s_par[PAR_BPROJ + e] = L.proj.bias[e]; s_par[PAR_BFF2 + e] = L.ff2.bias[e];
    }
    for (uint32_t e = tid; e < 768; e += 512) s_par[PAR_BQKV + e] = L.qkv.bias[e];
    for (uint32_t e = tid; e < d_ff; e += 512) s_par[PAR_BFF1 + e] = L.ff1.bias[e];
  };
  auto layer_norm = [&](uint32_t og, uint32_t ob, const float* __restrict__ gp, const float* __restrict__ bp, int want_lo) {
    float mean[PT], rstd[PT];
#pragma unroll
    for (int pass = 0; pass < 2; pass++) {
      float* red = s_red + pass * 8 * HLT;
#pragma unroll
      for (int pt = 0; pt < PT; pt++) {
        float sm = 0.f;
#pragma unroll
        for (int q = 0; q < 8; q++) {
          const float d = pass == 0 ? XQ(pt, q) : XQ(pt, q) - mean[pt];
          sm += pass == 0 ? d : d * d;
        }
        sm = fg_sum(sm);
        if (fg == 0) red[wave * HLT + pt * 16 + fr] = sm;
      }
      __syncthreads();
#pragma unroll
      for (int pt = 0; pt < PT; pt++) {
        float sm = 0.f;
#pragma unroll
        for (int w = 0; w < 8; w++) sm += red[w * HLT + pt * 16 + fr];
        if (pass == 0) mean[pt] = sm * (1.0f / 256.f);
        else rstd[pt] = __builtin_amdgcn_rsqf(sm * (1.0f / 256.f) + eps);
      }
    }
    float gg[8], bb[8];
    if (gp) {
      const float4 g0 = *reinterpret_cast<const float4*>(gp + cw + 8 * fg), g1 = *reinterpret_cast<const float4*>(gp + cw + 8 * fg + 4);
      const float4 b0 = *reinterpret_cast<const float4*>(bp + cw + 8 * fg), b1 = *reinterpret_cast<const float4*>(bp + cw + 8 * fg + 4);
      gg[0] = g0.x; gg[1] = g0.y; gg[2] = g0.z; gg[3] = g0.w; gg[4] = g1.x; gg[5] = g1.y; gg[6] = g1.z; gg[7] = g1.w;
      bb[0] = b0.x; bb[1] = b0.y; bb[2] = b0.z; bb[3] = b0.w; bb[4] = b1.x; bb[5] = b1.y; bb[6] = b1.z; bb[7] = b1.w;
    } else {
      lds8(og + cw + 8 * fg, gg);
      lds8(ob + cw + 8 * fg, bb);
    }
#pragma unroll
    for (int pt = 0; pt < PT; pt++) {
      float y[8];
#pragma unroll
      for (int q = 0; q < 8; q++) y[q] = (XQ(pt, q) - mean[pt]) * rstd[pt] * gg[q] + bb[q];
      const uint32_t o = hlsw(pt * 16 + fr, wave * 4 + fg);
      if (want_lo == 2 && (HERRO_LP_DBG & 16)) {
        *reinterpret_cast<half8*>(s_hh + o) = pack_h8(y);
      } else if (want_lo == 2) {
        half8 hi;
        uint2 lo8;
        split_h8_f8(y, hi, lo8);
        *reinterpret_cast<half8*>(s_hh + o) = hi;
        *reinterpret_cast<uint2*>(reinterpret_cast<uint8_t*>(s_hl) + lsw8(pt * 16 + fr, wave * 2 + (fg >> 1)) + (fg & 1u) * 8) = lo8;
      } else if (want_lo) {
        half8 hi, lo;
        split_h8(y, hi, lo);
        *reinterpret_cast<half8*>(s_hh + o) = hi;
        *reinterpret_cast<half8*>(s_hl + o) = lo;
      } else {
        *reinterpret_cast<half8*>(s_hh + o) = pack_h8(y);
      }
    }
    __syncthreads();
  };
  auto zero = [](f32x4 (&a)[PT][2]) {
#pragma unroll
    for (int pt = 0; pt < PT; pt++)
#pragma unroll
      for (int jt = 0; jt < 2; jt++) a[pt][jt] = f32x4{0.f, 0.f, 0.f, 0.f};
  };
  auto store_act = [&](auto terms_c, uint16_t* ph, uint16_t* pl, uint32_t o, const float (&v)[8]) {
    constexpr int TA = decltype(terms_c)::value;
    if (TA == 3 && (HERRO_LP_DBG & 16)) {
      *reinterpret_cast<half8*>(ph + o) = pack_h8(v);
    } else if (TA == 3) {
      half8 hi;
      uint2 lo8;
      split_h8_f8(v, hi, lo8);
      *reinterpret_cast<half8*>(ph + o) = hi;
      const uint32_t row = o >> 8, ch8 = ((o >> 3) & 31u) ^ (row & 15u);
      *reinterpret_cast<uint2*>(reinterpret_cast<uint8_t*>(pl) + lsw8(row, ch8 >> 1) + (ch8 & 1u) * 8) = lo8;
    } else if (TA == 2) {
      half8 hi, lo;
      split_h8(v, hi, lo);
      *reinterpret_cast<half8*>(ph + o) = hi;
      *reinterpret_cast<half8*>(pl + o) = lo;
    } else {
      *reinterpret_cast<half8*>(ph + o) = pack_h8(v);
    }
  };

  stage_params(M.layer[0]);
  {
    const float4 pdv = *reinterpret_cast<const float4*>(M.pe_div + ((cw + 8 * fg) >> 1));
    const float pd[4] = {pdv.x, pdv.y, pdv.z, pdv.w};
#pragma unroll
    for (int pt = 0; pt < PT; pt++) {
      const uint32_t tok = pt * 16 + fr;
      float4 a = make_float4(0.f, 0.f, 0.f, 0.f), b = a;
      float row = 0.f;
      uint32_t rowu = 0;
      if (tok < nt) {
        const float* xp = S.x + (uint64_t)(t0 + tok) * 256 + cw + 8 * fg;
        a = *reinterpret_cast<const float4*>(xp);
        b = *reinterpret_cast<const float4*>(xp + 4);
        rowu = S.tok_row[t0 + tok];
        row = (float)rowu;
      }
      xr[pt][0] = f32x4{a.x, a.y, a.z, a.w};
      xr[pt][1] = f32x4{b.x, b.y, b.z, b.w};
      if (tok < nt) {
        if (rowu >= M.pe_rows) {
#pragma unroll
          for (int j = 0; j < 4; j++) {
            const float ang = __fmul_rn(row, pd[j]);
            float sn, cs;
            sincosf(ang, &sn, &cs);
            xr[pt][j >> 1][(2 * j) & 3] += sn;
            xr[pt][j >> 1][(2 * j + 1) & 3] += cs;
          }
        }
      }
    }
  }
  __syncthreads();

  const float scale = 1.4426950408889634f / sqrtf(32.f);
  for (uint32_t li = 0; li < n_layers; li++) {
    const LayerW& L = M.layer[li];
    const LayerW& Ln = M.layer[li + 1 < n_layers ? li + 1 : 0];
    RELAUNDER();
    LP_MARK(li ? 7 : 0);
    layer_norm(PAR_LN1G, PAR_LN1B, nullptr, nullptr, 0);
    LP_MARK(1);
    RELAUNDER();
    {
      half8 qh[PT], kh[PT], vh[2][PT / 2];
      {
        f32x4 a[PT][2];
        float bq[8];
        zero(a);
        tile_gemm_p<false, 1, PT>(wstream(L.qkv, cw, 0, lane), wa, wstream(L.qkv, 256 + cw, 0, lane), s_hh, s_hl, fr, fg, a);
        lds8(PAR_BQKV + cw + 8 * fg, bq);
#pragma unroll
        for (int pt = 0; pt < PT; pt++) {
          float v[8];
#pragma unroll
          for (int q = 0; q < 8; q++) v[q] = (a[pt][q >> 2][q & 3] + bq[q]) * scale;
          qh[pt] = pack_h8(v);
        }
        zero(a);
        tile_gemm_p<false, 1, PT>(wstream(L.qkv, 256 + cw, 0, lane), wa, wstream(L.qkv, 512 + cw, 0, lane), s_hh, s_hl, fr, fg, a);
        lds8(PAR_BQKV + 256 + cw + 8 * fg, bq);
#pragma unroll
        for (int pt = 0; pt < PT; pt++) {
          float v[8];
#pragma unroll
          for (int q = 0; q < 8; q++) v[q] = a[pt][q >> 2][q & 3] + bq[q];
          kh[pt] = pack_h8(v);
        }
        zero(a);
        tile_gemm_p<true, 1, PT>(wstream(L.qkv, 512 + cw, 0, lane), wa, wstream(L.proj, cw, 0, lane), s_hh, s_hl, fr, fg, a);
#pragma unroll
        for (int ct = 0; ct < 2; ct++) {
          const float bv = s_par[PAR_BQKV + 512 + cw + 8 * (fr >> 2) + 4 * ct + (fr & 3)];
#pragma unroll
          for (int kk = 0; kk < PT / 2; kk++) {
            float v[8];
#pragma unroll
            for (int e = 0; e < 8; e++) v[e] = a[2 * kk + (e >> 2)][ct][e & 3] + bv;
            vh[ct][kk] = pack_h8(v);
          }
        }
      }
      LP_MARK(2);
      uint32_t wj[PT][4];
#pragma unroll
      for (int pj = 0; pj < PT; pj++)
#pragma unroll
        for (int r = 0; r < 4; r++) wj[pj][r] = s_win[pj * 16 + 4 * fg + r];
      if (!SIB || !big) {
#pragma unroll
      for (int pi = 0; pi < PT; pi++) {
        const uint32_t wi = s_win[pi * 16 + fr];
        f32x4 st[PT];
        float m = -INFINITY;
#pragma unroll
        for (int pj = 0; pj < PT; pj++) {
          st[pj] = mma(kh[pj], qh[pi], f32x4{0.f, 0.f, 0.f, 0.f});
#pragma unroll
          for (int r = 0; r < 4; r++) {
            st[pj][r] = wj[pj][r] == wi ? st[pj][r] : -INFINITY;
            m = fmax_nc(m, st[pj][r]);
          }
        }
        m = fg_max(m);
        float l = 0.f;
#pragma unroll
        for (int pj = 0; pj < PT; pj++) {
#pragma unroll
          for (int r = 0; r < 4; r++) {
            const float pexp = __builtin_amdgcn_exp2f(st[pj][r] - m);
            st[pj][r] = pexp;
            l += pexp;
          }
        }
        l = fg_sum(l);
        f32x4 o[2] = {f32x4{0.f, 0.f, 0.f, 0.f}, f32x4{0.f, 0.f, 0.f, 0.f}};
#pragma unroll
        for (int kk = 0; kk < PT / 2; kk++) {
          float v[8];
#pragma unroll
          for (int e = 0; e < 8; e++) v[e] = st[2 * kk + (e >> 2)][e & 3];
          const half8 ph = pack_h8(v);
#pragma unroll
          for (int ct = 0; ct < 2; ct++) o[ct] = mma(vh[ct][kk], ph, o[ct]);
        }
        const float inv = __builtin_amdgcn_rcpf(l);
        float v[8];
#pragma unroll
        for (int e = 0; e < 8; e++) v[e] = o[e >> 2][e & 3] * inv;
        store_act(std::integral_constant<int, TP>{}, s_ah, s_al, hlsw(pi * 16 + fr, wave * 4 + fg), v);
      }
      } else {
        {
          uint16_t* mine = S.sib_kv + ((((uint64_t)bt * 2 + (li & 1u)) * 8 + wave) * 8 * 64 + lane) * 8;
#pragma unroll
          for (int pt = 0; pt < PT; pt++) *reinterpret_cast<half8*>(mine + pt * 512) = kh[pt];
#pragma unroll
          for (int ct = 0; ct < 2; ct++)
#pragma unroll
            for (int kk = 0; kk < PT / 2; kk++) *reinterpret_cast<half8*>(mine + (PT + ct * (PT / 2) + kk) * 512) = vh[ct][kk];
          __builtin_amdgcn_fence(__ATOMIC_RELEASE, "agent");
          __syncthreads();
          if (tid == 0) __hip_atomic_store(S.sib_flag + bt, li + 1u, __ATOMIC_RELAXED, __HIP_MEMORY_SCOPE_AGENT);
        }
        float mrun[PT], lrun[PT];
        f32x4 orun[PT][2];
#pragma unroll
        for (int pi = 0; pi < PT; pi++) {
          const uint32_t wi = s_win[pi * 16 + fr];
          f32x4 st[PT];
          float m = -INFINITY;
#pragma unroll
          for (int pj = 0; pj < PT; pj++) {
            st[pj] = mma(kh[pj], qh[pi], f32x4{0.f, 0.f, 0.f, 0.f});
#pragma unroll
            for (int r = 0; r < 4; r++) {
              st[pj][r] = wj[pj][r] == wi ? st[pj][r] : -INFINITY;
              m = fmax_nc(m, st[pj][r]);
            }
          }
          m = fg_max(m);
          float l = 0.f;
#pragma unroll
          for (int pj = 0; pj < PT; pj++)
#pragma unroll
            for (int r = 0; r < 4; r++) {
              const float pexp = __builtin_amdgcn_exp2f(st[pj][r] - m);
              st[pj][r] = pexp;
              l += pexp;
            }
          mrun[pi] = m;
          lrun[pi] = fg_sum(l);
          orun[pi][0] = f32x4{0.f, 0.f, 0.f, 0.f};
          orun[pi][1] = f32x4{0.f, 0.f, 0.f, 0.f};
#pragma unroll
          for (int kk = 0; kk < PT / 2; kk++) {
            float v[8];
#pragma unroll
            for (int e = 0; e < 8; e++) v[e] = st[2 * kk + (e >> 2)][e & 3];
            const half8 ph = pack_h8(v);
#pragma unroll
            for (int ct = 0; ct < 2; ct++) orun[pi][ct] = mma(vh[ct][kk], ph, orun[pi][ct]);
          }
        }
        const uint32_t g0 = grp & 0xfffffu, gk = (grp >> 20) & 15u, nlast = grp >> 24;
        const uint32_t nbig = bt == g0 + gk - 1 ? nlast : (uint32_t)HLT;
#pragma unroll 1
        for (uint32_t sb = g0; sb < g0 + gk; sb++) {
          if (sb == bt) continue;
          uint32_t spins = 0;
          while (__hip_atomic_load(S.sib_flag + sb, __ATOMIC_RELAXED, __HIP_MEMORY_SCOPE_AGENT) <= li) {
            __builtin_amdgcn_s_sleep(16);
            if (++spins > (1u << 21)) {
              if (lane == 0) atomicExch(S.sib_err, 1u + li);
              break;
            }
          }
          __builtin_amdgcn_fence(__ATOMIC_ACQUIRE, "agent");
          const uint32_t nts = sb == g0 + gk - 1 ? nlast : (uint32_t)HLT;
          const uint16_t* src = S.sib_kv + ((((uint64_t)sb * 2 + (li & 1u)) * 8 + wave) * 8 * 64 + lane) * 8;
          half8 kf[PT], vf[2][PT / 2];
#pragma unroll
          for (int pt = 0; pt < PT; pt++) kf[pt] = *reinterpret_cast<const half8*>(src + pt * 512);
#pragma unroll
          for (int ct = 0; ct < 2; ct++)
#pragma unroll
            for (int kk = 0; kk < PT / 2; kk++) vf[ct][kk] = *reinterpret_cast<const half8*>(src + (PT + ct * (PT / 2) + kk) * 512);
#pragma unroll
          for (int pi = 0; pi < PT; pi++) {
            f32x4 st[PT];
            float bm = -INFINITY;
#pragma unroll
            for (int pj = 0; pj < PT; pj++) {
              st[pj] = mma(kf[pj], qh[pi], f32x4{0.f, 0.f, 0.f, 0.f});
#pragma unroll
              for (int r = 0; r < 4; r++) {
                st[pj][r] = ((uint32_t)(pj * 16 + 4 * fg + r) < nts && (uint32_t)(pi * 16) + fr < nbig) ? st[pj][r] : -INFINITY;
                bm = fmax_nc(bm, st[pj][r]);
              }
            }
            const float mn = fmax_nc(mrun[pi], fg_max(bm));
            const float alpha = __builtin_amdgcn_exp2f(mrun[pi] - mn);
            float l = 0.f;
#pragma unroll
            for (int pj = 0; pj < PT; pj++)
#pragma unroll
              for (int r = 0; r < 4; r++) {
                const float pexp = __builtin_amdgcn_exp2f(st[pj][r] - mn);
                st[pj][r] = pexp;
                l += pexp;
              }
            lrun[pi] = lrun[pi] * alpha + fg_sum(l);
            mrun[pi] = mn;
#pragma unroll
            for (int ct = 0; ct < 2; ct++)
#pragma unroll
              for (int r = 0; r < 4; r++) orun[pi][ct][r] *= alpha;
#pragma unroll
            for (int kk = 0; kk < PT / 2; kk++) {
              float v[8];
#pragma unroll
              for (int e = 0; e < 8; e++) v[e] = st[2 * kk + (e >> 2)][e & 3];
              const half8 ph = pack_h8(v);
#pragma unroll
              for (int ct = 0; ct < 2; ct++) orun[pi][ct] = mma(vf[ct][kk], ph, orun[pi][ct]);
            }
          }
        }
#pragma unroll
        for (int pi = 0; pi < PT; pi++) {
          const float inv = __builtin_amdgcn_rcpf(lrun[pi]);
          float v[8];
#pragma unroll
          for (int e = 0; e < 8; e++) v[e] = orun[pi][e >> 2][e & 3] * inv;
          store_act(std::integral_constant<int, TP>{}, s_ah, s_al, hlsw(pi * 16 + fr, wave * 4 + fg), v);
        }
      }
    }
    __syncthreads();
    LP_MARK(3);
    RELAUNDER();
    {
      float bp[8];
      lds8(PAR_BPROJ + cw + 8 * fg, bp);
#pragma unroll
      for (int pt = 0; pt < PT; pt++)
#pragma unroll
        for (int q = 0; q < 8; q++) XQ(pt, q) += bp[q];
      tile_gemm_p<false, TP, PT>(wstream<TP == 3>(L.proj, cw, 0, lane), wa, wstream(L.ff1, cw, 0, lane), s_ah, s_al, fr, fg, xr);
    }
    RELAUNDER();
    LP_MARK(4);
    layer_norm(PAR_LN2G, PAR_LN2B, nullptr, nullptr, TF == 3 ? 2 : (TF == 2 ? 1 : 0));
    LP_MARK(5);
    {
      {
        float b2[8];
        lds8(PAR_BFF2 + cw + 8 * fg, b2);
#pragma unroll
        for (int pt = 0; pt < PT; pt++)
#pragma unroll
          for (int q = 0; q < 8; q++) XQ(pt, q) += b2[q];
      }
      constexpr bool TWO_BUF = TF == 1;
      for (uint32_t c = 0; c < d_ff; c += 256) {
        RELAUNDER();
        uint16_t* hid = (TWO_BUF && ((c >> 8) & 1u)) ? s_al : s_ah;
        f32x4 a1[PT][2];
        {
          float b1[8];
          lds8(PAR_BFF1 + c + cw + 8 * fg, b1);
#pragma unroll
          for (int pt = 0; pt < PT; pt++)
#pragma unroll
            for (int jt = 0; jt < 2; jt++) a1[pt][jt] = f32x4{b1[4 * jt], b1[4 * jt + 1], b1[4 * jt + 2], b1[4 * jt + 3]};
        }
        tile_gemm_p<false, TF, PT>(wstream<TF == 3>(L.ff1, c + cw, 0, lane), wa, wstream(L.ff2, cw, c, lane), s_hh, s_hl, fr, fg, a1);
        LP_MARK(9);
#pragma unroll
        for (int pt = 0; pt < PT; pt++) {
          float v[8];
#pragma unroll
          for (int q = 0; q < 8; q++) v[q] = __builtin_amdgcn_fmed3f(a1[pt][q >> 2][q & 3], 0.f, __builtin_huge_valf());
          store_act(std::integral_constant<int, TF>{}, hid, s_al, hlsw(pt * 16 + fr, wave * 4 + fg), v);
        }
        LP_MARK(10);
        __syncthreads();
        LP_MARK(6);
        const bool more = c + 256 < d_ff;
        const WStream nx = more ? wstream(L.ff1, c + 256 + cw, 0, lane) : wstream(Ln.qkv, cw, 0, lane);
        tile_gemm_p<false, TF, PT>(wstream<TF == 3>(L.ff2, cw, c, lane), wa, nx, hid, s_al, fr, fg, xr);
        LP_MARK(11);
        if (!TWO_BUF || !more) __syncthreads();
        LP_MARK(7);
      }
    }
    if (li + 1 < n_layers) stage_params(Ln);
  }
  RELAUNDER();
  const uint64_t out_o = (wave < PT && wave * 16 + fr < nt) ? S.tok_out[t0 + wave * 16 + fr] : 0ull;
  const float4 hb = *reinterpret_cast<const float4*>(M.heads.bias + 4 * fg);
  layer_norm(0, 0, M.lnf_g, M.lnf_b, 1);
#undef RELAUNDER
#undef XQ
  if (wave < PT) {
    const uint32_t pt = wave;
    f32x4 a = f32x4{0.f, 0.f, 0.f, 0.f};
    const Weight& W = M.heads;
#pragma unroll
    for (int ks = 0; ks < 8; ks++) {
      const half8 wh = *reinterpret_cast<const half8*>(W.h16 + (uint64_t)fr * 256 + ks * 32 + fg * 8);
      const half8 wl = *reinterpret_cast<const half8*>(W.l16 + (uint64_t)fr * 256 + ks * 32 + fg * 8);
      const uint32_t o = hlsw(pt * 16 + fr, ks * 4 + fg);
      const half8 xh = *reinterpret_cast<const half8*>(s_hh + o);
      const half8 xl = *reinterpret_cast<const half8*>(s_hl + o);
      a = mma(wl, xh, a);
      a = mma(wh, xl, a);
      a = mma(wh, xh, a);
    }
    const uint32_t tok = pt * 16 + fr;
    if (tok < nt) {
      const uint64_t o = out_o;
      const float hbv[4] = {hb.x, hb.y, hb.z, hb.w};
#pragma unroll
      for (int r = 0; r < 4; r++) {
        const uint32_t ch = 4 * fg + r;
        const float v = a[r] + hbv[r];
        if (ch == 0) B.out_info[o] = v;
        else if (ch < 6) B.out_base[o * 5 + (ch - 1)] = v;
      }
    }
  }
  LP_MARK(8);
}
constexpr size_t layers_p_shm(int tokens) { return (size_t)4 * tokens * 256 * 2 + 2 * 8 * tokens * 4 + tokens * 4 + (size_t)PAR_FLOATS * 4; }

__global__ void k_build_tokens_h(BatchDev B, ModelScratch S) {
  const uint32_t b = blockIdx.x;
  const uint32_t t0 = B.tok_off[b], t1 = B.tok_off[b + 1];
  for (uint32_t n = t0 + threadIdx.x; n < t1; n += blockDim.x) {
    const uint32_t row = B.sup_row[B.sup_off[b] + (n - t0)];
    S.tok_win[n] = b;
    S.tok_row[n] = row;
    S.tok_out[n] = B.out_off[b] + (n - t0);
    TokMeta tm;
    tm.plane_off = B.plane_off[b];
    tm.plane_ld = B.plane_ld[b];
    tm.tok_row = row;
    tm.len = B.len[b];
    tm.lmax = B.lmax[b];
    tm.rf_idx = (uint32_t)((B.rf_base ? B.rf_base[b] : B.out_off[b]) + (n - t0));
    tm.pad1 = 0;
    S.tok_meta[n] = tm;
    uint32_t mk[2] = {0, 0}, dt[2] = {0, 0}, dq[2] = {0, 0}, ok = 0;
    for (int i = 0; i < 5; i++) {
      const int32_t r = (int32_t)row - 2 + i;
      const bool in = r >= 0 && r < (int32_t)tm.lmax, real = in && r < (int32_t)tm.len;
      const uint32_t sh = 8u * (i & 3);
      if (real) mk[i >> 2] |= 0xffu << sh;
      else { dt[i >> 2] |= (in ? (uint32_t)TOK_PAD : 12u) << sh; dq[i >> 2] |= (in ? 126u : 0xffu) << sh; }
    }
    for (int j = 0; j < 3; j++) {
      const int32_t pos = (int32_t)row + j - 1;
      if (pos >= 0 && pos < (int32_t)tm.lmax) ok |= 1u << j;
    }
    TokCv cv;
    cv.plane_off = tm.plane_off;
    cv.ld_d1 = (dt[1] << 16) | (dq[1] << 24);
    cv.row_ok = (ok << 16) | (mk[1] << 24);
    cv.rf_idx = tm.rf_idx;
    cv.mk0 = mk[0]; cv.dt0 = dt[0]; cv.dq0 = dq[0];
    S.tok_cv[n] = cv;
  }
}

__global__ void k_pe_table(const float* __restrict__ pe_div, float* __restrict__ tab, uint32_t rows, uint32_t half_d) {
  const uint32_t i = blockIdx.x * blockDim.x + threadIdx.x;
  if (i >= rows * half_d) return;
  const uint32_t row = i / half_d, j = i % half_d;
  const float ang = __fmul_rn((float)row, pe_div[j]);
  float sn, cs;
  sincosf(ang, &sn, &cs);
  *reinterpret_cast<float2*>(tab + (uint64_t)row * (2 * half_d) + 2 * j) = make_float2(sn, cs);
}

}

void launch_pe_table(const float* pe_div, float* tab, uint32_t rows, uint32_t d_model, hipStream_t st) {
  const uint32_t n = rows * (d_model / 2);
  hipLaunchKernelGGL(k_pe_table, dim3((n + 255) / 256), dim3(256), 0, st, pe_div, tab, rows, d_model / 2);
}

bool model_h_supported(const ModelDev& M) {
  const ModelHyper& h = M.h;
  if (!(model_default_variant(M) && h.d_model == 256 && h.n_heads == 8 && h.d_ff % 256 == 0 && h.d_ff <= (uint32_t)PAR_MAX_FF && h.rows == HERRO_ROWS && M.heads.h16 && M.heads.l16)) return false;
  for (uint32_t l = 0; l < h.n_layers; l++)
    if (!M.layer[l].qkv.ph16 || !M.layer[l].proj.ph16 || !M.layer[l].ff1.ph16 || !M.layer[l].ff2.ph16) return false;
  return true;
}

bool model_h_conv_supported(const ModelDev& M) {
  const ModelHyper& h = M.h;
  return h.kw == 3 && h.c1 == 64 && h.c2 == HC2 && M.conv1g.ph16 && M.conv2.ph16 && M.fc.h16 && M.fc.ph16 && M.fc.K % 128 == 0;
}

bool model_h_f8_supported(const ModelDev& M) {
  if (!model_h_supported(M)) return false;
  for (uint32_t l = 0; l < M.h.n_layers; l++)
    if (!M.layer[l].proj.p8 || !M.layer[l].ff1.p8 || !M.layer[l].ff2.p8) return false;
  return true;
}

int model_h_half_tiles(const ModelDev& M) {
  static const int mode = std::max(0, std::min(2, ab_env("HERRO_LAYERS_Q", 1)));
  return model_h_supported(M) ? mode : 0;
}

void launch_model_h(const ModelDev& M, const BatchDev& B, const ModelScratch& S, int terms, hipStream_t st, KernelTimer* tm) {
  const uint32_t N = B.n_tok;
  if (N == 0 || B.n_tiles + B.n_tiles_q + B.n_tiles_b == 0) return;
  const ModelHyper& h = M.h;
  const bool f16_front = model_h_conv_supported(M);
  ModelDev M_enc = M;
  if (!f16_front) {
    launch_front_generic(M, B, S, st, tm);
    M_enc.pe_rows = 0xffffffffu;
  } else {
  KT_BEGIN(tm, "build_tokens", st);
  hipLaunchKernelGGL(k_build_tokens_h, dim3(B.n_win), dim3(64), 0, st, B, S);
  KT_END(tm, st);
  static const uint32_t chunk_tok = (uint32_t)std::max(0, ab_env("HERRO_CONV_CHUNK", 0)) & ~15u;
  static const int force_g = ab_env("HERRO_FC_G", 0);
  static const uint32_t n_cu = [] { int dev = 0, c = 0; (void)hipGetDevice(&dev); (void)hipDeviceGetAttribute(&c, hipDeviceAttributeMultiprocessorCount, dev); return (uint32_t)std::max(c, 1); }();
  const uint32_t n_rows = N * HERRO_ROWS;
  auto conv = [&](uint32_t t0, uint32_t t1) {
    const uint32_t unit0 = t0 * HERRO_ROWS / 16, n_units = (std::min(t1 * HERRO_ROWS, n_rows) + 15) / 16, nu = n_units - unit0;
    if (B.rf_q) {
      opt_in_lds(reinterpret_cast<const void*>(k_conv_m<1, 3, true>), CONV_M_SHM);
      hipLaunchKernelGGL((k_conv_m<1, 3, true>), dim3(std::min<uint32_t>((nu + 3) / 4, 768u)), dim3(CM_NT), CONV_M_SHM, st, M, B, S, n_rows, n_units, unit0);
    } else {
      opt_in_lds(reinterpret_cast<const void*>(k_conv_m<1, 3, false>), CONV_M_SHM);
      hipLaunchKernelGGL((k_conv_m<1, 3, false>), dim3(std::min<uint32_t>((nu + 3) / 4, 768u)), dim3(CM_NT), CONV_M_SHM, st, M, B, S, n_rows, n_units, unit0);
    }
  };
  auto fc = [&](uint32_t t0, uint32_t t1) {
    const uint32_t n = t1 - t0, lda = HERRO_ROWS * h.c2;
    auto busiest = [&](uint32_t rows) { const uint32_t wg = (n + rows - 1) / rows; return (uint64_t)((wg + n_cu - 1) / n_cu) * rows + (wg > 2 * n_cu ? 1u << 20 : 0u); };
    int nb = 8;
    for (int b = 7; b >= 4; b--) if (busiest(16u * b) < busiest(16u * nb)) nb = b;
    if (force_g == 3) nb = 6; else if (force_g == 4) nb = 8; else if (force_g == 14) nb = 4; else if (force_g >= 5 && force_g <= 8) nb = force_g;
    const uint16_t* A = S.y2_hi + (uint64_t)t0 * lda;
    float* C = S.x + (uint64_t)t0 * h.d_model;
    const uint32_t* rows = S.tok_row + t0;
    const dim3 grid((n + 16u * nb - 1) / (16u * nb));
    switch (nb) {
      case 4: hipLaunchKernelGGL(k_fc_r<4>, grid, dim3(512), FC_R_SHM, st, A, lda, M.fc, C, h.d_model, n, rows, M.pe_tab, M.pe_rows); break;
      case 5: hipLaunchKernelGGL(k_fc_r<5>, grid, dim3(512), FC_R_SHM, st, A, lda, M.fc, C, h.d_model, n, rows, M.pe_tab, M.pe_rows); break;
      case 6: hipLaunchKernelGGL(k_fc_r<6>, grid, dim3(512), FC_R_SHM, st, A, lda, M.fc, C, h.d_model, n, rows, M.pe_tab, M.pe_rows); break;
      case 7: hipLaunchKernelGGL(k_fc_r<7>, grid, dim3(512), FC_R_SHM, st, A, lda, M.fc, C, h.d_model, n, rows, M.pe_tab, M.pe_rows); break;
      default: hipLaunchKernelGGL(k_fc_r<8>, grid, dim3(512), FC_R_SHM, st, A, lda, M.fc, C, h.d_model, n, rows, M.pe_tab, M.pe_rows);
    }
  };
  if (chunk_tok && N > chunk_tok) {
    KT_BEGIN(tm, "conv_fused", st);
    for (uint32_t t0 = 0; t0 < N; t0 += chunk_tok) { conv(t0, std::min(N, t0 + chunk_tok)); fc(t0, std::min(N, t0 + chunk_tok)); }
    KT_END(tm, st);
  } else {
    KT_BEGIN(tm, "conv_fused", st);
    conv(0, N);
    KT_END(tm, st);
    KT_BEGIN(tm, "fc_gemm", st);
    fc(0, N);
    KT_END(tm, st);
  }
  }
  KT_BEGIN(tm, "layers_fused", st);
  auto launch = [&](auto kern, uint32_t n_tiles, int tokens) {
    opt_in_lds(reinterpret_cast<const void*>(kern), layers_p_shm(tokens));
    hipLaunchKernelGGL(kern, dim3(n_tiles), dim3(512), layers_p_shm(tokens), st, M_enc, B, S);
  };
  auto launch5 = [&](auto k1, auto k2, auto k3, auto k21, auto k12, uint32_t n_tiles, int tokens) {
    switch (terms) {
      case 3: launch(k3, n_tiles, tokens); break;
      case 2: launch(k2, n_tiles, tokens); break;
      case 21: launch(k21, n_tiles, tokens); break;
      case 12: launch(k12, n_tiles, tokens); break;
      default: launch(k1, n_tiles, tokens);
    }
  };
  if (B.n_tiles_b) {
    (void)hipMemsetAsync(S.sib_flag, 0, (size_t)B.n_tiles_b * 4, st);
    launch5(k_layers_p<1, 4, true>, k_layers_p<2, 4, true>, k_layers_p<3, 4, true>, k_layers_p<21, 4, true>, k_layers_p<12, 4, true>, B.n_tiles_b + B.n_tiles, 64);
  } else if (B.n_tiles) launch5(k_layers_p<1, 4>, k_layers_p<2, 4>, k_layers_p<3, 4>, k_layers_p<21, 4>, k_layers_p<12, 4>, B.n_tiles, 64);
  if (B.n_tiles_q) launch5(k_layers_p<1, 2>, k_layers_p<2, 2>, k_layers_p<3, 2>, k_layers_p<21, 2>, k_layers_p<12, 2>, B.n_tiles_q, 32);
  KT_END(tm, st);
}

#ifdef HERRO_PROF_BUILD
void model_h_prof_dump() {
  unsigned long long h[16] = {0};
  if (hipMemcpyFromSymbol(h, HIP_SYMBOL(g_lp_prof), sizeof h) != hipSuccess || !h[15]) return;
  static const char* name[12] = {"prologue", "LN1", "QKV", "attention", "proj", "LN2", "FF1 barrier wait", "FF2 barrier wait", "final LN + heads", "FF1 gemm", "FF1 epilogue", "FF2 gemm"};
  fprintf(stderr, "PROF k_layers_p (%llu tiles sampled), shader cycles per tile by phase:", h[15]);
  for (int p = 0; p < 12; p++) fprintf(stderr, " %s %.0f", name[p], (double)h[p] / (double)h[15]);
  fprintf(stderr, "\n");
}
#endif

}
```

### include/herro_amd.h

```cpp
#ifndef HERRO_AMD_H
#define HERRO_AMD_H

#include <stddef.h>
#include <stdint.h>

#ifdef __cplusplus
extern "C" {
#endif

#define HERRO_OK 0
#define HERRO_E_INVALID (-1)
#define HERRO_E_NO_DEVICE (-2)
#define HERRO_E_REFERENCE_PANIC (-3)
#define HERRO_E_UNSUPPORTED (-4)
#define HERRO_E_NO_MODEL (-5)
#define HERRO_E_STATE (-6)

#define HERRO_ROWS 31
#define HERRO_N_CLASSES 5

typedef struct herro_ctx herro_ctx;
typedef struct herro_job herro_job;

typedef struct {
// ... 20 lines not shown
void herro_destroy(herro_ctx* ctx);
const char* herro_last_error(const herro_ctx* ctx);
int herro_set_stream(herro_ctx* ctx, void* hip_stream);
int herro_synchronize(herro_ctx* ctx);

int64_t herro_encode_2bit(const uint8_t* seq, uint64_t n, uint64_t* words);
int herro_decode_2bit(const uint64_t* words, uint64_t length, uint64_t start, uint64_t end,
                      int reverse_complement, uint8_t* out);

int herro_set_reads(herro_ctx* ctx, uint32_t n_reads, const uint8_t* seq, const uint8_t* qual,
                    const uint64_t* off, const uint32_t* name_class);
int herro_set_reads_packed(herro_ctx* ctx, uint32_t n_reads, const uint64_t* words,
                           const uint64_t* word_off, const uint8_t* qual, const uint64_t* qual_off,
                           const uint32_t* name_class);
int herro_share_reads(herro_ctx* ctx, const herro_ctx* from);

int herro_load_model(herro_ctx* ctx, const char* path);
int herro_set_precision(herro_ctx* ctx, int mode);
int herro_precision(const herro_ctx* ctx);
int herro_clock_probe(herro_ctx* ctx, double* shader_mhz);
float herro_calibration_error(const herro_ctx* ctx, int mode);

int64_t herro_model_describe(const herro_ctx* ctx, char* out, uint64_t cap);

herro_job* herro_job_create(herro_ctx* ctx, uint32_t n_targets, const uint32_t* rids,
                            const uint64_t* aln_off, const herro_alignment* alns,
                            uint32_t window_size);
void herro_job_free(herro_job* job);
int herro_host_register(herro_ctx* ctx, const void* p, uint64_t bytes);
int herro_host_unregister(herro_ctx* ctx, const void* p);
uint64_t herro_debug_zero_copy_jobs(void);
int herro_job_create_status(const herro_ctx* ctx);
uint32_t herro_job_n_windows(const herro_job* job);
int herro_job_skipped(const herro_job* job, uint32_t* n_alignments, uint32_t* n_targets);

int herro_job_featurize(herro_job* job);

int herro_job_infer(herro_job* job, uint32_t batch_size, int batch_mode);

int herro_job_window_info(herro_job* job, uint32_t w, herro_window_info* info);
int herro_job_window_copy(herro_job* job, uint32_t w, int encoded, uint8_t* bases, uint8_t* quals,
                          uint16_t* sup_pos, uint8_t* sup_ins, uint32_t* qids);
int herro_job_window_logits(herro_job* job, uint32_t w, float* info_logits, float* bases_logits);

int herro_job_consensus(herro_job* job);

int herro_job_consensus_fetch(herro_job* job, uint64_t* n_bases);

int64_t herro_job_consensus_fasta(herro_job* job, uint32_t t, const char* id, const char* desc,
                                  char* out, uint64_t cap);

int64_t herro_job_fasta(herro_job* job, const char* const* ids, const char* const* descs, char* out, uint64_t cap,
                        uint64_t* rec_end);

int herro_model_forward(herro_ctx* ctx, uint32_t B, uint32_t L, const uint8_t* bases,
                        const uint8_t* quals, const int32_t* lens, const int32_t* indices,
                        float* info_logits, float* bases_logits);

int herro_timing_enable(herro_ctx* ctx, int on);
int herro_timing_reset(herro_ctx* ctx);
int herro_timing_get(herro_ctx* ctx, char* names, uint64_t names_cap, double* ms, uint64_t* calls,
                     uint32_t* n);
int herro_job_stats(herro_job* job, uint64_t* out);

int64_t herro_debug_extract_windows(const herro_alignment* a, uint32_t n_windows, uint32_t window_size,
                                    uint64_t* out, uint64_t cap, char* err, uint64_t err_cap);

herro_ctx* herro_debug_host_ctx(uint32_t n_reads, const uint32_t* read_len, const uint32_t* name_class);
int64_t herro_debug_job_array(herro_job* job, int which, const void** ptr, uint32_t* elem_bytes);

int herro_debug_set_featurize_planes(herro_ctx* ctx, int on);
int herro_debug_set_host_build(herro_ctx* ctx, int on);
int herro_debug_job_dev_built(const herro_job* job);
int herro_debug_base_row_votes(const uint8_t* counts, const uint8_t* split, const uint8_t* target, uint32_t n, uint8_t* sup, uint8_t* vote);
uint32_t herro_debug_vote5(const uint32_t* c5, uint32_t tb);
int64_t herro_debug_job_rf(herro_job* job, uint32_t w, uint8_t* out, uint64_t cap);
int64_t herro_debug_job_cwd(herro_job* job, uint32_t ow, uint32_t* out, uint64_t cap);
int herro_debug_job_rf_fused(const herro_job* job);
int herro_debug_job_rf_left(const herro_job* job);
uint32_t herro_debug_e4m3(float x);
int herro_debug_sib_fault(herro_ctx* ctx);
int herro_debug_force_precision(herro_ctx* ctx, int on);
int herro_debug_sib_retries(const herro_ctx* ctx);
int herro_debug_job_set_base_logits(herro_job* job, const float* base, uint64_t n_rows);

int64_t herro_debug_tile_plan(const uint32_t* cnt, uint32_t n, int packed, uint32_t n_cu, uint32_t* order, uint32_t* n_half, uint32_t* tile_tok);
int herro_debug_tile_plan_sib(const uint32_t* cnt, uint32_t n, int packed, uint32_t n_cu, uint32_t* order, uint32_t* n_tiles,
                              uint32_t* tile_tok, uint32_t* grp);

typedef struct herro_paf herro_paf;
typedef struct herro_name_index herro_name_index;
herro_name_index* herro_name_index_create(uint32_t n_reads, const char* names, const uint64_t* name_off);
void herro_name_index_free(herro_name_index* index);
herro_paf* herro_paf_parse_indexed(const char* text, uint64_t len, const herro_name_index* index, const uint8_t* core,
                                   int n_threads, char* err, uint64_t err_cap);
herro_paf* herro_oec_read_indexed(const char* path, const herro_name_index* index, const uint8_t* core, int n_threads,
                                  char* err, uint64_t err_cap);
herro_paf* herro_paf_parse_view(const char* text, uint64_t len, const herro_name_index* index, const uint8_t* core,
                                int n_threads, char* err, uint64_t err_cap);
herro_paf* herro_paf_parse(const char* text, uint64_t len, uint32_t n_reads, const char* names,
                           const uint64_t* name_off, const uint8_t* core, int n_threads, char* err,
                           uint64_t err_cap);
herro_paf* herro_oec_read(const char* path, uint32_t n_reads, const char* names, const uint64_t* name_off,
                          const uint8_t* core, int n_threads, char* err, uint64_t err_cap);
herro_paf* herro_paf_parse_coords(const char* text, uint64_t len, const herro_name_index* index, const uint8_t* core, int n_threads,
                                  char* err, uint64_t err_cap);
uint32_t herro_paf_n_targets(const herro_paf* p);
const uint32_t* herro_paf_target_ids(const herro_paf* p);
const uint64_t* herro_paf_aln_off(const herro_paf* p);
const herro_alignment* herro_paf_alignments(const herro_paf* p);
void herro_paf_free(herro_paf* p);

#define HERRO_ALIGN_BAND 128
typedef struct herro_aligned herro_aligned;
int herro_align_overlaps(herro_ctx* ctx, uint32_t n, const herro_alignment* in, herro_aligned** out);
const herro_alignment* herro_aligned_alignments(const herro_aligned* a);
const int32_t* herro_aligned_scores(const herro_aligned* a);
uint32_t herro_aligned_failed(const herro_aligned* a);
void herro_aligned_free(herro_aligned* a);

typedef struct herro_aligned_dev herro_aligned_dev;
int herro_align_overlaps_dev(herro_ctx* ctx, uint32_t n, const herro_alignment* in, herro_aligned_dev** out);
int herro_aligned_dev_from_ops(herro_ctx* ctx, uint32_t n, const herro_alignment* alns, const uint64_t* op_off ,
                               const uint32_t* ops, herro_aligned_dev** out);
int herro_aligned_dev_mirror(herro_ctx* ctx, const herro_aligned_dev* src, herro_aligned_dev** out);
uint32_t herro_aligned_dev_n(const herro_aligned_dev* a);
const herro_alignment* herro_aligned_dev_alignments(const herro_aligned_dev* a);
const int32_t* herro_aligned_dev_scores(const herro_aligned_dev* a);
const uint32_t* herro_aligned_dev_n_ops(const herro_aligned_dev* a);
uint32_t herro_aligned_dev_failed(const herro_aligned_dev* a);
int64_t herro_aligned_dev_cigar(const herro_aligned_dev* a, uint32_t r, char* out, uint64_t cap);
void herro_aligned_dev_free(herro_aligned_dev* a);
herro_job* herro_job_create_aligned(herro_ctx* ctx, uint32_t n_targets, const uint32_t* rids, const uint64_t* aln_off,
                                    const uint32_t* rec, const herro_aligned_dev* a, uint32_t window_size);

typedef struct { uint32_t zdrop, max_ext, reserved[2]; } herro_extend_params;
typedef struct herro_extended herro_extended;
int herro_extend_overlaps(herro_ctx* ctx, uint32_t n, const herro_alignment* in, const herro_extend_params* params ,
                          herro_extended** out);
uint32_t herro_extended_n(const herro_extended* x);
const herro_alignment* herro_extended_alignments(const herro_extended* x);
const uint32_t* herro_extended_ext(const herro_extended* x);
const int32_t* herro_extended_scores(const herro_extended* x);
void herro_extended_free(herro_extended* x);

typedef struct { uint32_t k, w, max_occ, bandwidth, max_gap, min_score, min_anchors, reserved; } herro_overlap_params;
typedef struct herro_overlaps herro_overlaps;
int herro_find_overlaps(herro_ctx* ctx, const herro_overlap_params* params , herro_overlaps** out);
uint32_t herro_overlaps_n(const herro_overlaps* o);
uint32_t herro_overlaps_n_targets(const herro_overlaps* o);
const uint32_t* herro_overlaps_target_ids(const herro_overlaps* o);
const uint64_t* herro_overlaps_aln_off(const herro_overlaps* o);
const herro_alignment* herro_overlaps_alignments(const herro_overlaps* o);
const int32_t* herro_overlaps_scores(const herro_overlaps* o);
void herro_overlaps_free(herro_overlaps* o);
typedef struct herro_pairs herro_pairs;
#define HERRO_PAIRS_NO_EXTEND 1u
int herro_find_overlap_pairs(herro_ctx* ctx, const herro_overlap_params* params ,
                             const herro_extend_params* extend_params , uint32_t flags, herro_pairs** out);
int herro_pairs_from_table(herro_ctx* ctx, uint32_t n_pairs, const herro_alignment* primaries, const int32_t* chain_scores, uint32_t n_targets,
                           const uint32_t* rids, const uint64_t* aln_off , const uint32_t* rec_of_row ,
                           herro_pairs** out);
int herro_pairs_align(herro_ctx* ctx, const herro_pairs* pairs, herro_aligned_dev** out);
herro_job* herro_job_create_paired(herro_ctx* ctx, const herro_pairs* pairs, const herro_aligned_dev* m, uint32_t window_size);
uint32_t herro_pairs_n(const herro_pairs* pairs);
const herro_alignment* herro_pairs_primaries(const herro_pairs* pairs);
const int32_t* herro_pairs_chain_scores(const herro_pairs* pairs);
const uint32_t* herro_pairs_ext(const herro_pairs* pairs);
const int32_t* herro_pairs_ext_scores(const herro_pairs* pairs);
uint32_t herro_pairs_n_targets(const herro_pairs* pairs);
const uint32_t* herro_pairs_target_ids(const herro_pairs* pairs);
// ... 52 lines not shown
```

Before: 3.255 million windows/s.

## Add 80-token fused-layer tiles with cost-model plan selection for single-term tier

Adds an 80-token tile height (PT=5) to the fused transformer-layer kernel for the single-term fp16 tier, aliasing the low-precision plane in LDS so the taller tile fits. The tile planner now builds both a 64-token plan and 80-token variants, scores each by a per-height cost model over rounds of CU-sized waves, and keeps the cheapest. This aims to cut wave-quantisation tail rounds and raise per-CU work at the price of larger LDS use, possibly lower occupancy, and padded V blocks when PT is odd. It also adds debug hooks for planning CU count and counting tall launches.

```diff
diff --git a/herro_amd/api.py b/herro_amd/api.py
--- a/herro_amd/api.py
+++ b/herro_amd/api.py
@@ -20,7 +20,7 @@
     "herro_timing_get", "herro_job_stats", "herro_debug_extract_windows",
     "herro_paf_parse", "herro_oec_read", "herro_paf_n_targets", "herro_paf_target_ids", "herro_paf_aln_off",
     "herro_paf_alignments", "herro_paf_free", "herro_name_index_create", "herro_name_index_free", "herro_paf_parse_indexed",
-    "herro_oec_read_indexed", "herro_paf_parse_view", "herro_debug_host_ctx", "herro_debug_job_array", "herro_debug_tile_plan", "herro_debug_tile_plan_sib",
+    "herro_oec_read_indexed", "herro_paf_parse_view", "herro_debug_host_ctx", "herro_debug_job_array", "herro_debug_tile_plan", "herro_debug_tile_plan_sib", "herro_debug_tile_plan_tall", "herro_debug_set_plan_cus", "herro_debug_tall_launches",
     "herro_debug_set_featurize_planes", "herro_debug_set_host_build", "herro_debug_job_dev_built", "herro_debug_job_rf", "herro_debug_job_cwd", "herro_debug_job_set_base_logits", "herro_debug_job_rf_fused", "herro_debug_job_rf_left", "herro_debug_e4m3", "herro_debug_sib_fault", "herro_debug_sib_retries", "herro_debug_base_row_votes", "herro_debug_vote5",
     "herro_pool_create", "herro_pool_destroy", "herro_pool_last_error", "herro_pool_size", "herro_pool_ctx", "herro_pool_set_reads", "herro_pool_load_model",
     "herro_pool_correct", "herro_pool_result", "herro_pool_groups_taken", "herro_pool_skipped", "herro_debug_pool_fake", "herro_job_create_status", "herro_host_register", "herro_host_unregister", "herro_debug_zero_copy_jobs",
@@ -293,6 +293,15 @@
         L.herro_debug_tile_plan.argtypes = [vp, u32, i32, u32, vp, vp, vp]
         L.herro_debug_tile_plan_sib.restype = i32
         L.herro_debug_tile_plan_sib.argtypes = [vp, u32, i32, u32, vp, vp, vp, vp]
+        try:
+            L.herro_debug_tile_plan_tall.restype = i32
+            L.herro_debug_tile_plan_tall.argtypes = [vp, u32, i32, u32, vp, vp, vp]
+            L.herro_debug_set_plan_cus.argtypes = [vp, u32]
+            L.herro_debug_tall_launches.restype = C.c_int64
+            L.herro_debug_tall_launches.argtypes = [vp]
+        except AttributeError:
+            if not os.environ.get("HERRO_LIB"):
+                raise
         _LIB = L
     return _LIB
 
@@ -352,6 +361,19 @@
         raise HerroError(int(rc), "herro_debug_tile_plan_sib")
     nb, n64, n32 = (int(x) for x in n_tiles)
     return nb, n64, n32, order[:len(c)], tok[:nb + n64 + n32 + 1], grp[:nb]
+
+
+def debug_tile_plan_tall(counts, packed: bool = True, n_cu: int = 256):
+    c = np.ascontiguousarray(counts, np.uint32)
+    order = np.zeros(max(len(c), 1), np.uint32)
+    cap = int(((c.astype(np.int64) + 63) // 64).sum()) + 2
+    n_tiles = np.zeros(4, np.uint32)
+    tok = np.zeros(cap, np.uint32)
+    rc = lib().herro_debug_tile_plan_tall(c.ctypes.data, len(c), int(packed), n_cu, order.ctypes.data, n_tiles.ctypes.data, tok.ctypes.data)
+    if rc < 0:
+        raise HerroError(int(rc), "herro_debug_tile_plan_tall")
+    nb, nh, n32, height = (int(x) for x in n_tiles)
+    return nb, nh, n32, height, order[:len(c)], tok[:nb + nh + n32 + 1]
 
 
 class Pool:
@@ -730,6 +752,12 @@
 
     def sib_retries(self) -> int:
         return int(self._l.herro_debug_sib_retries(self.h))
+
+    def set_plan_cus(self, n: int):
+        self._chk(self._l.herro_debug_set_plan_cus(self.h, int(n)))
+
+    def tall_launches(self) -> int:
+        return int(self._l.herro_debug_tall_launches(self.h))
 
     def timing_enable(self, on: bool = True):
         self._chk(self._l.herro_timing_enable(self.h, int(on)))
diff --git a/herro_amd/csrc/api_ctx.h b/herro_amd/csrc/api_ctx.h
--- a/herro_amd/csrc/api_ctx.h
+++ b/herro_amd/csrc/api_ctx.h
@@ -95,6 +95,8 @@
 struct herro_ctx {
   int device = 0;
   uint32_t n_cu = 256;
+  uint32_t plan_cu = 0;
+  uint64_t n_tall_launch = 0;
   hipStream_t own_stream = nullptr, stream = nullptr;
   ErrSlot err;
   uint32_t n_reads = 0;
diff --git a/herro_amd/csrc/herro_api.hip b/herro_amd/csrc/herro_api.hip
--- a/herro_amd/csrc/herro_api.hip
+++ b/herro_amd/csrc/herro_api.hip
@@ -235,21 +235,40 @@
     while (top && by[top].empty()) top--;
   }
 }
-static std::vector<uint32_t> tile_pack_order(const std::vector<uint32_t>& cnt) {
-  std::vector<std::vector<uint32_t>> by(FUSED_MAX_TOK + 1);
-  for (size_t i = cnt.size(); i-- > 0;) by[std::min(cnt[i], FUSED_MAX_TOK)].push_back((uint32_t)i);
+static std::vector<uint32_t> tile_pack_order(const std::vector<uint32_t>& cnt, uint32_t cap = FUSED_MAX_TOK) {
+  std::vector<std::vector<uint32_t>> by(cap + 1);
+  for (size_t i = cnt.size(); i-- > 0;) by[std::min(cnt[i], cap)].push_back((uint32_t)i);
   std::vector<uint32_t> order;
   order.reserve(cnt.size());
   for (uint32_t i : by[0]) order.push_back(i);
-  tile_pack_bins(cnt, by, cnt.size() - by[0].size(), FUSED_MAX_TOK, order);
+  tile_pack_bins(cnt, by, cnt.size() - by[0].size(), cap, order);
   return order;
 }
 
-struct TilePlan { std::vector<uint32_t> order, tiles, tiles_q, tiles_b, grp; };
-static TilePlan plan_tiles_small(const std::vector<uint32_t>& cnt, bool pack, int qmode, uint32_t n_cu, uint32_t n_busy = 0);
+struct TilePlan { std::vector<uint32_t> order, tiles, tiles_q, tiles_b, grp; uint32_t tile_h = 64; };
+static constexpr double TILE_COST_32 = 0.68, TILE_COST_80 = 1.31;
+static TilePlan plan_tiles_small(const std::vector<uint32_t>& cnt, bool pack, int qmode, uint32_t n_cu, uint32_t n_busy = 0, uint32_t cap = FUSED_MAX_TOK, bool any_tail = false);
+static double plan_cost(const TilePlan& P, uint32_t n_cu) {
+  const uint32_t cu = std::max(n_cu, 1u);
+  auto rounds = [&](const std::vector<uint32_t>& t) { return t.empty() ? 0.0 : (double)((t.size() - 1 + cu - 1) / cu); };
+  return rounds(P.tiles) * (P.tile_h == FUSED_TALL_TOK ? TILE_COST_80 : 1.0) + rounds(P.tiles_q) * TILE_COST_32;
+}
 static TilePlan plan_tiles(const std::vector<uint32_t>& cnt, bool pack, int qmode, uint32_t n_cu) {
   std::vector<uint32_t> big, small;
   for (size_t i = 0; i < cnt.size(); i++) (cnt[i] > FUSED_MAX_TOK ? big : small).push_back((uint32_t)i);
+  if (qmode >= 3) {
+    if (!big.empty()) return plan_tiles(cnt, pack, 1, n_cu);
+    TilePlan best = plan_tiles_small(cnt, pack, 1, n_cu);
+    if (cnt.empty()) return best;
+    double cost = qmode == 4 ? 1e300 : plan_cost(best, n_cu);
+    for (int tail = 0; tail < (qmode == 4 ? 1 : 2); tail++) {
+      TilePlan T = plan_tiles_small(cnt, pack, tail, n_cu, 0, FUSED_TALL_TOK, true);
+      if (T.tiles.empty()) continue;
+      const double c = plan_cost(T, n_cu);
+      if (c < cost) { cost = c; best = std::move(T); }
+    }
+    return best;
+  }
   if (big.empty()) return plan_tiles_small(cnt, pack, qmode, n_cu);
   std::vector<std::vector<uint32_t>> by(FUSED_MAX_TOK + 1);
   if (pack) for (size_t k = small.size(); k-- > 0;) by[cnt[small[k]]].push_back(small[k]);
@@ -287,24 +306,26 @@
   P.grp.swap(grp);
   return P;
 }
-static TilePlan plan_tiles_small(const std::vector<uint32_t>& cnt, bool pack, int qmode, uint32_t n_cu, uint32_t n_busy) {
+static TilePlan plan_tiles_small(const std::vector<uint32_t>& cnt, bool pack, int qmode, uint32_t n_cu, uint32_t n_busy, uint32_t cap, bool any_tail) {
   TilePlan P;
+  P.tile_h = cap;
   const size_t n = cnt.size();
   std::vector<uint32_t> tok_off(1, 0);
   auto finish = [&](size_t n_head) {
     tok_off.assign(1, 0);
     for (size_t k = 0; k < n; k++) tok_off.push_back(tok_off.back() + cnt[P.order[k]]);
-    P.tiles = token_tiles(tok_off, 0, n_head, FUSED_MAX_TOK);
+    P.tiles = token_tiles(tok_off, 0, n_head, cap);
     P.tiles_q.clear();
     if (n_head < n) P.tiles_q = token_tiles(tok_off, n_head, n, FUSED_HALF_TOK);
   };
   if (qmode != 2) {
-    if (pack) P.order = tile_pack_order(cnt);
+    if (pack) P.order = tile_pack_order(cnt, cap);
     else { P.order.resize(n); for (size_t i = 0; i < n; i++) P.order[i] = (uint32_t)i; }
     finish(n);
     const size_t n64 = P.tiles.empty() ? 0 : P.tiles.size() - 1;
-    const size_t rr = n_cu ? (n64 + n_busy) % n_cu : 0;
-    if (qmode == 0 || rr == 0 || 2 * rr > n_cu) return P;
+    size_t rr = n_cu ? (n64 + n_busy) % n_cu : 0;
+    if (any_tail && rr == 0 && n64) rr = n_cu;
+    if (qmode == 0 || rr == 0 || (!any_tail && 2 * rr > n_cu)) return P;
     const size_t r = std::min(rr, n64);
     if (r == 0) return P;
     const uint32_t cut_tok = P.tiles[n64 - r];
@@ -411,11 +432,18 @@
   if (threadIdx.x == 0) { out[0] = c1 - c0; out[1] = w1 - w0; out[2] = x; }
 }
 
+static int h_terms(int p) { return p == 4 ? 2 : (p == 6 ? 3 : (p == 7 ? 21 : (p == 8 ? 12 : 1))); }
+static int fused_qmode(const herro_ctx* ctx) {
+  if (ctx->precision < 4) return 0;
+  const int tall = model_h_tall_tiles(ctx->M, h_terms(ctx->precision));
+  return tall ? 2 + tall : model_h_half_tiles(ctx->M);
+}
 static void run_model(herro_ctx* ctx, const BatchDev& B, bool tiled) {
   if (B.n_tok == 0) return;
   const int p = ctx->precision;
+  if (tiled && p >= 4 && B.n_tiles && B.tile_h == FUSED_TALL_TOK) ctx->n_tall_launch++;
   if (!tiled) { launch_model(ctx->M, B, ctx->S, (p == 1 || p >= 4) ? 3 : p, ctx->stream, &ctx->timer); return; }
-  if (p >= 4) launch_model_h(ctx->M, B, ctx->S, p == 4 ? 2 : (p == 6 ? 3 : (p == 7 ? 21 : (p == 8 ? 12 : 1))), ctx->stream, &ctx->timer);
+  if (p >= 4) launch_model_h(ctx->M, B, ctx->S, h_terms(p), ctx->stream, &ctx->timer);
   else launch_model(ctx->M, B, ctx->S, p, ctx->stream, &ctx->timer);
 }
 
@@ -2089,12 +2117,13 @@
     std::memcpy(blob.data() + o, p, bytes);
     return o;
   };
-  struct Offs { size_t plane_off, plane_ld, len, lmax, tok_off, sup_off, out_off, rf_base, tiles, tiles_q, tiles_b, grp; uint32_t n_tiles, n_tiles_q, n_tiles_b, n_win, n_tok, max_win_tok; bool tiled; };
+  struct Offs { size_t plane_off, plane_ld, len, lmax, tok_off, sup_off, out_off, rf_base, tiles, tiles_q, tiles_b, grp; uint32_t n_tiles, n_tiles_q, n_tiles_b, n_win, n_tok, max_win_tok, tile_h; bool tiled; };
   std::vector<Offs> offs;
   uint32_t max_tok = 0, max_tiles_b = 0;
   const bool fused_mode = ctx->precision == 1 || ctx->precision >= 4;
   const uint32_t tok_cap = job->no_sib ? FUSED_MAX_TOK : fused_tok_cap(ctx);
-  const int qmode = ctx->precision >= 4 ? model_h_half_tiles(ctx->M) : 0;
+  const int qmode = fused_qmode(ctx);
+  const uint32_t plan_cu = ctx->plan_cu ? ctx->plan_cu : ctx->n_cu;
   for (auto& g : groups) {
     for (int part = 0; part < 2; part++) {
       std::vector<uint64_t> plane_off, sup_o, out_o, rfb;
@@ -2112,7 +2141,7 @@
       const size_t B = sel.size();
       if (B == 0) continue;
       TilePlan plan;
-      if (fused_mode && part == 0) plan = plan_tiles(sel_cnt, ctx->tile_packing, qmode, ctx->n_cu);
+      if (fused_mode && part == 0) plan = plan_tiles(sel_cnt, ctx->tile_packing, qmode, plan_cu);
       const std::vector<uint32_t>& order = plan.order;
       plane_off.reserve(B); sup_o.reserve(B); out_o.reserve(B); ld.reserve(B); len.reserve(B); lmax.reserve(B); tok_off.reserve(B + 1);
       for (size_t k = 0; k < B; k++) {
@@ -2132,6 +2161,7 @@
       o.tok_off = put(tok_off.data(), (B + 1) * 4);
       o.sup_off = put(sup_o.data(), B * 8); o.out_off = put(out_o.data(), B * 8); o.rf_base = put(rfb.data(), B * 8);
       o.n_tiles = plan.tiles.empty() ? 0u : (uint32_t)plan.tiles.size() - 1;
+      o.tile_h = plan.tile_h;
       o.tiles = put(plan.tiles.data(), plan.tiles.size() * 4);
       o.n_tiles_q = plan.tiles_q.empty() ? 0u : (uint32_t)plan.tiles_q.size() - 1;
       o.tiles_q = put(plan.tiles_q.data(), plan.tiles_q.size() * 4);
@@ -2183,6 +2213,7 @@
     B.rf_base = (const uint64_t*)(base + o.rf_base);
     B.n_tiles = o.n_tiles;
     B.tile_tok0 = (const uint32_t*)(base + o.tiles);
+    B.tile_h = o.tile_h;
     B.n_tiles_q = o.n_tiles_q;
     B.tile_tok0_q = (const uint32_t*)(base + o.tiles_q);
     B.n_tiles_b = o.n_tiles_b;
@@ -2640,7 +2671,7 @@
       sel.push_back(b);
       sel_cnt.push_back((uint32_t)lens[b]);
     }
-    if (tiled) P.plan = plan_tiles(sel_cnt, ctx->tile_packing, ctx->precision >= 4 ? model_h_half_tiles(ctx->M) : 0, ctx->n_cu);
+    if (tiled) P.plan = plan_tiles(sel_cnt, ctx->tile_packing, fused_qmode(ctx), ctx->plan_cu ? ctx->plan_cu : ctx->n_cu);
     const std::vector<uint32_t>& order = P.plan.order;
     for (size_t k = 0; k < sel.size(); k++) {
       const uint32_t b = sel[order.empty() ? k : order[k]];
@@ -2658,6 +2689,7 @@
     bd.sup_off = (const uint64_t*)up(P.sup_off.data(), nb * 8); bd.out_off = (const uint64_t*)up(P.out_off.data(), nb * 8);
     bd.tile_tok0 = (const uint32_t*)up(P.plan.tiles.data(), P.plan.tiles.size() * 4);
     bd.n_tiles = P.plan.tiles.empty() ? 0u : (uint32_t)P.plan.tiles.size() - 1;
+    bd.tile_h = P.plan.tile_h;
     bd.tile_tok0_q = (const uint32_t*)up(P.plan.tiles_q.data(), P.plan.tiles_q.size() * 4);
     bd.n_tiles_q = P.plan.tiles_q.empty() ? 0u : (uint32_t)P.plan.tiles_q.size() - 1;
     bd.tile_tok0_b = (const uint32_t*)up(P.plan.tiles_b.data(), P.plan.tiles_b.size() * 4);
@@ -2750,6 +2782,12 @@
   return HERRO_OK;
 }
 int herro_debug_sib_retries(const herro_ctx* ctx) { return ctx ? (int)ctx->n_sib_retry : HERRO_E_INVALID; }
+int herro_debug_set_plan_cus(herro_ctx* ctx, uint32_t n) {
+  if (!ctx) return HERRO_E_INVALID;
+  ctx->plan_cu = n;
+  return HERRO_OK;
+}
+int64_t herro_debug_tall_launches(const herro_ctx* ctx) { return ctx ? (int64_t)ctx->n_tall_launch : HERRO_E_INVALID; }
 
 int herro_clock_probe(herro_ctx* ctx, double* shader_mhz) {
   if (!ctx || !shader_mhz) return HERRO_E_INVALID;
@@ -2875,6 +2913,29 @@
     tile_tok[k] = n32 ? P.tiles_q.back() : (n64 ? P.tiles.back() : 0);
   }
   return (int64_t)n64;
+}
+
+int herro_debug_tile_plan_tall(const uint32_t* cnt, uint32_t n, int packed, uint32_t n_cu, uint32_t* order, uint32_t* n_tiles, uint32_t* tile_tok) {
+  if (!cnt || !order || !n_tiles) return HERRO_E_INVALID;
+  std::vector<uint32_t> c(cnt, cnt + n);
+  for (uint32_t v : c) if (v == 0 || v > FUSED_MAX_TOK * FUSED_MAX_SIB) return HERRO_E_INVALID;
+  const TilePlan P = plan_tiles(c, (packed & 1) != 0, 3, n_cu);
+  for (uint32_t i = 0; i < n; i++) order[i] = P.order[i];
+  const size_t nb = P.grp.size(), nh = P.tiles.empty() ? 0 : P.tiles.size() - 1, n32 = P.tiles_q.empty() ? 0 : P.tiles_q.size() - 1;
+  if (nb && (P.tiles_b.size() != nb + 1 || P.tile_h != FUSED_MAX_TOK)) return HERRO_E_STATE;
+  n_tiles[0] = (uint32_t)nb; n_tiles[1] = (uint32_t)nh; n_tiles[2] = (uint32_t)n32; n_tiles[3] = P.tile_h;
+  if (tile_tok) {
+    size_t k = 0;
+    uint32_t end = 0;
+    for (size_t i = 0; i < nb; i++) tile_tok[k++] = P.tiles_b[i];
+    if (nb) end = P.tiles_b.back();
+    for (size_t i = 0; i < nh; i++) tile_tok[k++] = P.tiles[i];
+    if (nh) end = P.tiles.back();
+    for (size_t i = 0; i < n32; i++) tile_tok[k++] = P.tiles_q[i];
+    if (n32) end = P.tiles_q.back();
+    tile_tok[k] = end;
+  }
+  return HERRO_OK;
 }
 
 int herro_debug_tile_plan_sib(const uint32_t* cnt, uint32_t n, int packed, uint32_t n_cu, uint32_t* order, uint32_t* n_tiles, uint32_t* tile_tok, uint32_t* grp) {
diff --git a/herro_amd/csrc/model_dev.h b/herro_amd/csrc/model_dev.h
--- a/herro_amd/csrc/model_dev.h
+++ b/herro_amd/csrc/model_dev.h
@@ -78,6 +78,7 @@
   const uint32_t* sup_row;
   uint32_t n_tiles;
   const uint32_t* tile_tok0;
+  uint32_t tile_h;
   uint32_t n_tiles_q;
   const uint32_t* tile_tok0_q;
   uint32_t n_tiles_b;
@@ -134,6 +135,8 @@
 bool model_h_conv_supported(const ModelDev& M);
 void launch_front_generic(const ModelDev& M, const BatchDev& B, const ModelScratch& S, hipStream_t st, KernelTimer* tm);
 bool model_h_f8_supported(const ModelDev& M);
+constexpr uint32_t FUSED_TALL_TOK = 80;
+int model_h_tall_tiles(const ModelDev& M, int terms);
 int model_h_half_tiles(const ModelDev& M);
 void launch_model_h(const ModelDev& M, const BatchDev& B, const ModelScratch& S, int terms, hipStream_t st, KernelTimer* tm);
 void launch_pe_table(const float* pe_div, float* tab, uint32_t rows, uint32_t d_model, hipStream_t st);
diff --git a/herro_amd/csrc/model_h.hip b/herro_amd/csrc/model_h.hip
--- a/herro_amd/csrc/model_h.hip
+++ b/herro_amd/csrc/model_h.hip
@@ -627,8 +627,10 @@
   constexpr int HLT = 16 * PT;
   extern __shared__ __attribute__((aligned(16))) unsigned char smem[];
   uint16_t* s_hh = reinterpret_cast<uint16_t*>(smem);
+  static_assert(PT != 5 || TERMS == 1, "80-token tiles: the single-term tier only (the lo plane is aliased)");
+  constexpr bool ALIAS_HL = PT == 5;
   uint16_t* s_hl = s_hh + HLT * 256;
-  uint16_t* s_ah = s_hl + HLT * 256;
+  uint16_t* s_ah = ALIAS_HL ? s_hl : s_hl + HLT * 256;
   uint16_t* s_al = s_ah + HLT * 256;
   float* s_red = reinterpret_cast<float*>(s_al + HLT * 256);
   uint32_t* s_win = reinterpret_cast<uint32_t*>(s_red + 2 * 8 * HLT);
@@ -636,7 +638,7 @@
   const uint32_t tid = threadIdx.x, lane = tid & 63, wave = __builtin_amdgcn_readfirstlane(tid >> 6);
   LP_BEGIN();
   uint32_t fr = lane & 15, fg = lane >> 4;
-  const uint32_t* tile_tok0 = PT == 4 ? (big ? B.tile_tok0_b : B.tile_tok0) : B.tile_tok0_q;
+  const uint32_t* tile_tok0 = PT == 2 ? B.tile_tok0_q : (big ? B.tile_tok0_b : B.tile_tok0);
   const uint32_t t0 = tile_tok0[bt], nt = tile_tok0[bt + 1] - t0;
   const uint32_t grp = big ? B.tile_grp[bt] : 0u;
   const uint32_t cw = wave * 32;
@@ -799,7 +801,8 @@
     LP_MARK(1);
     RELAUNDER();
     {
-      half8 qh[PT], kh[PT], vh[2][PT / 2];
+      constexpr int NV = (PT + 1) / 2;
+      half8 qh[PT], kh[PT], vh[2][NV];
       {
         f32x4 a[PT][2];
         float bq[8];
@@ -829,10 +832,13 @@
         for (int ct = 0; ct < 2; ct++) {
           const float bv = s_par[PAR_BQKV + 512 + cw + 8 * (fr >> 2) + 4 * ct + (fr & 3)];
 #pragma unroll
-          for (int kk = 0; kk < PT / 2; kk++) {
+          for (int kk = 0; kk < NV; kk++) {
             float v[8];
 #pragma unroll
-            for (int e = 0; e < 8; e++) v[e] = a[2 * kk + (e >> 2)][ct][e & 3] + bv;
+            for (int e = 0; e < 8; e++) {
+              const int blk = 2 * kk + (e >> 2);
+              v[e] = blk < PT ? a[blk < PT ? blk : 0][ct][e & 3] + bv : 0.f;
+            }
             vh[ct][kk] = pack_h8(v);
           }
         }
@@ -872,10 +878,13 @@
         l = fg_sum(l);
         f32x4 o[2] = {f32x4{0.f, 0.f, 0.f, 0.f}, f32x4{0.f, 0.f, 0.f, 0.f}};
 #pragma unroll
-        for (int kk = 0; kk < PT / 2; kk++) {
+        for (int kk = 0; kk < NV; kk++) {
           float v[8];
 #pragma unroll
-          for (int e = 0; e < 8; e++) v[e] = st[2 * kk + (e >> 2)][e & 3];
+          for (int e = 0; e < 8; e++) {
+            const int blk = 2 * kk + (e >> 2);
+            v[e] = blk < PT ? st[blk < PT ? blk : 0][e & 3] : 0.f;
+          }
           const half8 ph = pack_h8(v);
 #pragma unroll
           for (int ct = 0; ct < 2; ct++) o[ct] = mma(vh[ct][kk], ph, o[ct]);
@@ -894,7 +903,7 @@
 #pragma unroll
           for (int ct = 0; ct < 2; ct++)
 #pragma unroll
-            for (int kk = 0; kk < PT / 2; kk++) *reinterpret_cast<half8*>(mine + (PT + ct * (PT / 2) + kk) * 512) = vh[ct][kk];
+            for (int kk = 0; kk < NV; kk++) *reinterpret_cast<half8*>(mine + (PT + ct * NV + kk) * 512) = vh[ct][kk];
           __builtin_amdgcn_fence(__ATOMIC_RELEASE, "agent");
           __syncthreads();
           if (tid == 0) __hip_atomic_store(S.sib_flag + bt, li + 1u, __ATOMIC_RELAXED, __HIP_MEMORY_SCOPE_AGENT);
@@ -930,10 +939,13 @@
           orun[pi][0] = f32x4{0.f, 0.f, 0.f, 0.f};
           orun[pi][1] = f32x4{0.f, 0.f, 0.f, 0.f};
 #pragma unroll
-          for (int kk = 0; kk < PT / 2; kk++) {
+          for (int kk = 0; kk < NV; kk++) {
             float v[8];
 #pragma unroll
-            for (int e = 0; e < 8; e++) v[e] = st[2 * kk + (e >> 2)][e & 3];
+            for (int e = 0; e < 8; e++) {
+              const int blk = 2 * kk + (e >> 2);
+              v[e] = blk < PT ? st[blk < PT ? blk : 0][e & 3] : 0.f;
+            }
             const half8 ph = pack_h8(v);
 #pragma unroll
             for (int ct = 0; ct < 2; ct++) orun[pi][ct] = mma(vh[ct][kk], ph, orun[pi][ct]);
@@ -955,13 +967,13 @@
           __builtin_amdgcn_fence(__ATOMIC_ACQUIRE, "agent");
           const uint32_t nts = sb == g0 + gk - 1 ? nlast : (uint32_t)HLT;
           const uint16_t* src = S.sib_kv + ((((uint64_t)sb * 2 + (li & 1u)) * 8 + wave) * 8 * 64 + lane) * 8;
-          half8 kf[PT], vf[2][PT / 2];
+          half8 kf[PT], vf[2][NV];
 #pragma unroll
           for (int pt = 0; pt < PT; pt++) kf[pt] = *reinterpret_cast<const half8*>(src + pt * 512);
 #pragma unroll
           for (int ct = 0; ct < 2; ct++)
 #pragma unroll
-            for (int kk = 0; kk < PT / 2; kk++) vf[ct][kk] = *reinterpret_cast<const half8*>(src + (PT + ct * (PT / 2) + kk) * 512);
+            for (int kk = 0; kk < NV; kk++) vf[ct][kk] = *reinterpret_cast<const half8*>(src + (PT + ct * NV + kk) * 512);
 #pragma unroll
           for (int pi = 0; pi < PT; pi++) {
             f32x4 st[PT];
@@ -993,10 +1005,13 @@
 #pragma unroll
               for (int r = 0; r < 4; r++) orun[pi][ct][r] *= alpha;
 #pragma unroll
-            for (int kk = 0; kk < PT / 2; kk++) {
+            for (int kk = 0; kk < NV; kk++) {
               float v[8];
 #pragma unroll
-              for (int e = 0; e < 8; e++) v[e] = st[2 * kk + (e >> 2)][e & 3];
+              for (int e = 0; e < 8; e++) {
+                const int blk = 2 * kk + (e >> 2);
+                v[e] = blk < PT ? st[blk < PT ? blk : 0][e & 3] : 0.f;
+              }
               const half8 ph = pack_h8(v);
 #pragma unroll
               for (int ct = 0; ct < 2; ct++) orun[pi][ct] = mma(vf[ct][kk], ph, orun[pi][ct]);
@@ -1109,7 +1124,7 @@
   }
   LP_MARK(8);
 }
-constexpr size_t layers_p_shm(int tokens) { return (size_t)4 * tokens * 256 * 2 + 2 * 8 * tokens * 4 + tokens * 4 + (size_t)PAR_FLOATS * 4; }
+constexpr size_t layers_p_shm(int tokens, int planes = 4) { return (size_t)planes * tokens * 256 * 2 + 2 * 8 * tokens * 4 + tokens * 4 + (size_t)PAR_FLOATS * 4; }
 
 __global__ void k_build_tokens_h(BatchDev B, ModelScratch S) {
   const uint32_t b = blockIdx.x;
@@ -1190,6 +1205,10 @@
 int model_h_half_tiles(const ModelDev& M) {
   static const int mode = std::max(0, std::min(2, ab_env("HERRO_LAYERS_Q", 1)));
   return model_h_supported(M) ? mode : 0;
+}
+int model_h_tall_tiles(const ModelDev& M, int terms) {
+  static const int mode = std::max(0, std::min(2, ab_env("HERRO_LAYERS_TALL", 1)));
+  return (terms == 1 && model_h_half_tiles(M) == 1) ? mode : 0;
 }
 
 void launch_model_h(const ModelDev& M, const BatchDev& B, const ModelScratch& S, int terms, hipStream_t st, KernelTimer* tm) {
@@ -1251,9 +1270,9 @@
   }
   }
   KT_BEGIN(tm, "layers_fused", st);
-  auto launch = [&](auto kern, uint32_t n_tiles, int tokens) {
-    opt_in_lds(reinterpret_cast<const void*>(kern), layers_p_shm(tokens));
-    hipLaunchKernelGGL(kern, dim3(n_tiles), dim3(512), layers_p_shm(tokens), st, M_enc, B, S);
+  auto launch = [&](auto kern, uint32_t n_tiles, int tokens, int planes = 4) {
+    opt_in_lds(reinterpret_cast<const void*>(kern), layers_p_shm(tokens, planes));
+    hipLaunchKernelGGL(kern, dim3(n_tiles), dim3(512), layers_p_shm(tokens, planes), st, M_enc, B, S);
   };
   auto launch5 = [&](auto k1, auto k2, auto k3, auto k21, auto k12, uint32_t n_tiles, int tokens) {
     switch (terms) {
@@ -1267,6 +1286,9 @@
   if (B.n_tiles_b) {
     (void)hipMemsetAsync(S.sib_flag, 0, (size_t)B.n_tiles_b * 4, st);
     launch5(k_layers_p<1, 4, true>, k_layers_p<2, 4, true>, k_layers_p<3, 4, true>, k_layers_p<21, 4, true>, k_layers_p<12, 4, true>, B.n_tiles_b + B.n_tiles, 64);
+  } else if (B.n_tiles && B.tile_h == FUSED_TALL_TOK) {
+    if (terms != 1) { fprintf(stderr, "herro_amd: 80-token tiles planned for a tier without their kernel (terms %d)\n", terms); abort(); }
+    launch(k_layers_p<1, 5>, B.n_tiles, 80, 3);
   } else if (B.n_tiles) launch5(k_layers_p<1, 4>, k_layers_p<2, 4>, k_layers_p<3, 4>, k_layers_p<21, 4>, k_layers_p<12, 4>, B.n_tiles, 64);
   if (B.n_tiles_q) launch5(k_layers_p<1, 2>, k_layers_p<2, 2>, k_layers_p<3, 2>, k_layers_p<21, 2>, k_layers_p<12, 2>, B.n_tiles_q, 32);
   KT_END(tm, st);
diff --git a/include/herro_amd.h b/include/herro_amd.h
--- a/include/herro_amd.h
+++ b/include/herro_amd.h
@@ -126,11 +126,15 @@
 int herro_debug_sib_fault(herro_ctx* ctx);
 int herro_debug_force_precision(herro_ctx* ctx, int on);
 int herro_debug_sib_retries(const herro_ctx* ctx);
+int herro_debug_set_plan_cus(herro_ctx* ctx, uint32_t n);
+int64_t herro_debug_tall_launches(const herro_ctx* ctx);
 int herro_debug_job_set_base_logits(herro_job* job, const float* base, uint64_t n_rows);
 
 int64_t herro_debug_tile_plan(const uint32_t* cnt, uint32_t n, int packed, uint32_t n_cu, uint32_t* order, uint32_t* n_half, uint32_t* tile_tok);
 int herro_debug_tile_plan_sib(const uint32_t* cnt, uint32_t n, int packed, uint32_t n_cu, uint32_t* order, uint32_t* n_tiles,
                               uint32_t* tile_tok, uint32_t* grp);
+
+int herro_debug_tile_plan_tall(const uint32_t* cnt, uint32_t n, int packed, uint32_t n_cu, uint32_t* order, uint32_t* n_tiles, uint32_t* tile_tok);
 
 typedef struct herro_paf herro_paf;
 typedef struct herro_name_index herro_name_index;
```

Result: no change. 3.252 million windows/s (-0.1%).
